# zwpku/colvars-finder

Measured on AMD Instinct MI355X. Metric: MD frames/sec through EigenFunctionTask train step, higher is better.
Workload: dtype f32; 1 GPU; BASELINE config 3: alanine-dipeptide-shaped EigenFunctionTask, generator mode, k=3, 22 atoms, align+position features d_r=66, nets [66,20,20,20,1], diag_coeff, Adam; frames_per_gpu=100000, batch_per_gpu=20000, global_batch=20000, parallelism=dp1 (frames sharded; all-reduce of batch sums + flat gradient)

## Files before the change

### colvars-finder_amd/csrc/ef16_back.hip

```cpp
#include "ef16_common.hpp"

namespace {

struct Back16Args {
  int k;
  int64_t B;
  int64_t n_tiles;
  int64_t T;
  const float* w_lag;
};
struct Back16Nets {
  int D;
  int n_params;
  int base[CVF_MAX_NETS];
};
template <int H, int NH>
__host__ __device__ constexpr int net_w_off(int l, int hd) { return l == 0 ? 0 : hd + H + (l - 1) * (H * H + H); }
template <int H, int NH>
__host__ __device__ constexpr int net_b_off(int l, int hd) { return net_w_off<H, NH>(l, hd) + (l == 0 ? hd : l == NH ? H : H * H); }

template <int H, int NH, bool MULTI, bool GEN>
__global__ __launch_bounds__(256, 4) void ef16_back_kernel(Back16Args args, Back16Nets nets, const float* __restrict__ theta,
                                                            const float* __restrict__ packed, const float* __restrict__ w,
                                                            const float* __restrict__ feat, const float* __restrict__ y_tiled,
                                                            const float* __restrict__ q_tiled, const double* __restrict__ coef,
                                                            float* __restrict__ slab, int32_t* __restrict__ step,
                                                            const float* __restrict__ saved) {
  constexpr int RT = Hid<H>::RT, NG = Hid<H>::NG;
  constexpr int RTO = (H + 15) / 16;
  constexpr int CTH = (H + 1 + 15) / 16;
  constexpr int NT = 256, WPB = 4;
  constexpr bool TAIL4 = RTO == 2 && H % 16 >= 1 && H % 16 <= 4;
  constexpr int kRows = 2 * H + 2 * (H + 1) + 16;
  __shared__ __attribute__((aligned(16))) float IMG[kRows * kPitch];
  __shared__ float PART[4 * (H + 1)];
  extern __shared__ float GI[];
  float* SA1 = IMG;
  float* SA2 = SA1 + H * kPitch;
  float* SB1 = SA2 + H * kPitch;
  float* SB2 = SB1 + (H + 1) * kPitch;
  const int tid = threadIdx.x;
  const int wave = __builtin_amdgcn_readfirstlane(tid >> 6);
  int lane = tid & 63, col, q, row16, r0, fo, rowf;
  auto derive_lane = [&]() {
    col = lane & 15, q = lane >> 4, row16 = col, r0 = 4 * q;
    fo = 16 * wave + col;
    rowf = 4 * col + q;
  };
  derive_lane();
  static_assert(H % 4 == 0, "a lane's four rows of a gradient tile are inside the layer together (emit_tile)");
  const int net = blockIdx.y;
  int k = args.k;
  int D = nets.D, HD, c0, nfeat, ncol, CTM;
  bool strip;
  PackLayout L;
  auto derive = [&]() {
    const int CT1 = (D + 1 + 15) / 16;
    HD = H * D;
    c0 = 16 * (CT1 - 1), nfeat = D - c0, ncol = nfeat + 1;
    strip = ncol <= 4;
    CTM = strip ? CT1 - 1 : CT1;
    L = pack_layout(H, NH, D);
  };
  derive();
  const int gbase = nets.base[net];
  const int gspan = net_b_off<H, NH>(NH, HD) + 1;
  float* out = slab + (int64_t)blockIdx.x * nets.n_params + gbase;

  {
    static_assert((kRows * kPitch) % 4 == 0, "IMG is zeroed in 16-byte pieces");
    float4* img4 = reinterpret_cast<float4*>(IMG);
    for (int i = tid; i < kRows * kPitch / 4; i += NT) img4[i] = float4{0.0f, 0.0f, 0.0f, 0.0f};
  }
  if (MULTI)
    for (int i = tid; i < gspan; i += NT) GI[i] = 0.0f;
  lds_barrier();
  if (tid < 64) SB1[H * kPitch + tid] = 1.0f;

  const URows pk = urows(packed + (int64_t)net * L.per_net, L.per_net, lane);
  float wl[RT][4];
  load_hid_const_u<H>(urows(theta + gbase + net_w_off<H, NH>(NH, HD), H, q), wl);
  const float one[1] = {1.0f};

  const __amdgpu_buffer_rsrc_t out_rs = __builtin_amdgcn_make_buffer_rsrc(out, 0, gspan * 4, 0x00020000);
  constexpr int kDead = 0x7fff0000;
  auto emit_tile = [&](int l, int n_in, int rt, int ct, const f32x4& acc) {
    const int wo = net_w_off<H, NH>(l, HD), bo = net_b_off<H, NH>(l, HD);
    const int i = 16 * ct + row16;
    int ob = 16 * rt + r0;
    asm volatile("" : "+v"(ob));
    const bool isb = i == n_in, live = ob < H && i <= n_in;
    const int idx0 = isb ? bo + ob : wo + ob * n_in + i, stride = isb ? 1 : n_in;
    const int off0 = live ? idx0 * 4 : kDead;
#pragma unroll
    for (int r = 0; r < 4; ++r) {
      const float av = acc[r];
      if (MULTI) {
        if (live) GI[idx0 + r * stride] += av;
      } else {
        __builtin_amdgcn_raw_buffer_store_b32(__builtin_bit_cast(int, av), out_rs, off0 + r * stride * 4, 0, 0);
      }
    }
  };
  auto outer2 = [&](const float* A1, const float* B1, const float* A2, const float* B2, int rt, int ct) {
    f32x4 acc = {0.0f, 0.0f, 0.0f, 0.0f};
    acc = outer_half(A1, B1, rt, ct, lane, acc);
    if constexpr (GEN) acc = outer_half(A2, B2, rt, ct, lane, acc);
    return acc;
  };

  auto emit_entry = [&](bool live, int idx, float v) {
    if (MULTI) {
      if (live) GI[idx] += v;
    } else {
      __builtin_amdgcn_raw_buffer_store_b32(__builtin_bit_cast(int, v), out_rs, live ? idx * 4 : kDead, 0, 0);
    }
  };
  auto emit_last = [&]() {
    if (wave == WPB - 1) {
      int i = lane;
      asm volatile("" : "+v"(i));
      const bool live = i <= H;
      const float v = strip_total(PART + (live ? i : H), H + 1);
      emit_entry(live, i < H ? net_w_off<H, NH>(NH, HD) + i : net_b_off<H, NH>(NH, HD), v);
    }
  };
  auto emit_strip = [&]() {
    if (strip && 64 * wave < 4 * H) {
      int e = tid;
      asm volatile("" : "+v"(e));
      const int o = e >> 2, c = e & 3;
      const bool live = o < H && c < ncol;
      const float v = strip_total(SB1 + (o < H ? e : 0), 4 * H);
      emit_entry(live, c < nfeat ? o * D + c0 + c : HD + o, v);
    }
  };

  int64_t tile = blockIdx.x;
  do {
    if constexpr (MULTI) {
      asm volatile("" : "+s"(D), "+s"(k));
      derive();
      asm volatile("" : "+v"(lane));
      derive_lane();
    }
    CVF_STAMP(8);
    double crow[CVF_MAX_NETS];
#pragma unroll
    for (int j = 0; j < CVF_MAX_NETS; ++j) crow[j] = coef[k + net * k + (j < k ? j : k - 1)];
    double gS1n = coef[net], gEtn = coef[k + k * k + net];
    double gS1ln = GEN ? 0.0 : coef[2 * k + k * k + net], gS2ln = GEN ? 0.0 : coef[3 * k + k * k + net];
    __builtin_amdgcn_sched_barrier(0);
    const bool lagged = !GEN && tile >= args.T;
    const int64_t t0 = lagged ? tile - args.T : tile;
    const int64_t frame = t0 * CVF_TILE + fo;
    const bool valid = frame < args.B;
    const float wraw = w[valid ? frame : args.B - 1];
    float yb[CVF_MAX_NETS];
#pragma unroll
    for (int j = 0; j < CVF_MAX_NETS; ++j) yb[j] = y_tiled[(t0 * k + (j < k ? j : k - 1)) * CVF_TILE + fo];
    float ylag = 0.0f, wlraw = 0.0f;
    if constexpr (!GEN) {
      ylag = y_tiled[((args.T + t0) * k + net) * CVF_TILE + fo];
      wlraw = args.w_lag[valid ? frame : args.B - 1];
    }
    const URows sv = urows(saved + (tile * k + net) * (int64_t)(kHand<NH>() * NG * 256) + wave * 64, kHand<NH>() * NG * 256 - wave * 64, lane);
    Vec<H, 1> h[NH], e[NH > 1 ? NH - 1 : 1], t[NH];
#pragma unroll
    for (int l = 0; l < NH; ++l) {
#pragma unroll
      for (int rt = 0; rt < RT; ++rt) h[l].v[rt][0] = f32x4{0.0f, 0.0f, 0.0f, 0.0f};
#pragma unroll
      for (int g = 0; g < NG; ++g) h[l].v[g >> 2][0][g & 3] = sv.ld((l * NG + g) * 256);
    }
    if constexpr (GEN) {
#pragma unroll
      for (int l = 0; l + 1 < NH; ++l) {
#pragma unroll
        for (int rt = 0; rt < RT; ++rt) e[l].v[rt][0] = f32x4{0.0f, 0.0f, 0.0f, 0.0f};
#pragma unroll
        for (int g = 0; g < NG; ++g) e[l].v[g >> 2][0][g & 3] = sv.ld(((NH + l) * NG + g) * 256);
      }
#pragma unroll
      for (int rt = 0; rt < RT; ++rt) t[0].v[rt][0] = f32x4{0.0f, 0.0f, 0.0f, 0.0f};
#pragma unroll
      for (int g = 0; g < NG; ++g) t[0].v[g >> 2][0][g & 3] = sv.ld(((2 * NH - 1) * NG + g) * 256);
    }
    HFrag<H> ffr[NH > 1 ? NH - 1 : 1];
    if constexpr (GEN) {
#pragma unroll
      for (int l = 1; l < NH; ++l) load_hfrag_u<H>(ffr[l - 1], pk, L.fh(l));
    }
    const float* f_tile = feat + tile * (int64_t)D * CVF_TILE;
    const float* q_tile = GEN ? q_tiled + (tile * k + net) * (int64_t)D * CVF_TILE : nullptr;
    const float wb = valid ? wraw : 0.0f;
    float alpha, gamma = 0.0f;
    float ynet = 0.0f;
#pragma unroll
    for (int j = 0; j < CVF_MAX_NETS; ++j)
      if (j == net) ynet = yb[j];
#pragma unroll
    for (int j = 0; j < CVF_MAX_NETS; ++j) asm volatile("" : "+s"(crow[j]));
    asm volatile("" : "+s"(gS1n), "+s"(gEtn));
    if constexpr (!GEN) asm volatile("" : "+s"(gS1ln), "+s"(gS2ln));
    if (GEN || !lagged) {
      double a = gS1n;
#pragma unroll
      for (int j = 0; j < CVF_MAX_NETS; ++j)
        if (j < k) a += (j == net ? 2.0 : 1.0) * crow[j] * (double)yb[j];
      alpha = (float)((double)wb * a);
      if constexpr (GEN) gamma = (float)(2.0 * (double)wb * gEtn);
      else alpha = (float)((double)wb * a - 2.0 * (double)wb * gEtn * ((double)ylag - (double)ynet));
    } else {
      const double wlg = valid ? (double)wlraw : 0.0;
      alpha = (float)(wlg * (gS1ln + 2.0 * gS2ln * (double)ylag) + 2.0 * (double)wb * gEtn * ((double)ylag - (double)ynet));
    }
    CVF_STAMP(9);
    if constexpr (GEN) {
#pragma unroll
      for (int rt = 0; rt < RT; ++rt)
#pragma unroll
        for (int r = 0; r < 4; ++r) t[0].v[rt][0][r] *= gamma;
#pragma unroll
      for (int l = 1; l < NH; ++l) {
        Vec<H, 1> td;
        tangent_of<H, 1>(td, h[l - 1], t[l - 1]);
        init_bias<H, 1>(t[l], nullptr, q);
        hidden_mul<H, 1>(t[l], ffr[l - 1], td);
      }
    }
    CVF_STAMP(11);
    {
      const float pick = strip_rows<H>([&](int rt, int r) {
        const float hv = h[NH - 1].v[rt][0][r];
        if constexpr (GEN) return fmaf(alpha, hv, (1.0f - hv * hv) * t[NH - 1].v[rt][0][r]);
        else return alpha * hv;
      }, col);
      const float sa = row_sumf16(alpha);
      if (col < NG && rowf < H) PART[wave * (H + 1) + rowf] = pick;
      if (lane == 0) PART[wave * (H + 1) + H] = sa;
    }
    CVF_STAMP(12);
    Vec<H, 1> hbar;
#pragma unroll
    for (int rt = 0; rt < RT; ++rt)
#pragma unroll
      for (int r = 0; r < 4; ++r) hbar.v[rt][0][r] = alpha * wl[rt][r];
    HFrag<H> tfl;
    float4 bA[4], bB[4];
    float xs[3] = {0.0f, 0.0f, 0.0f}, qs[3] = {0.0f, 0.0f, 0.0f};
    auto request = [&](float4 (&dst)[4], const float* src_tile, int ct) {
      const int i = 16 * ct + row16;
      const float4* p = reinterpret_cast<const float4*>(src_tile + (int64_t)(i < D ? i : D - 1) * CVF_TILE + 4 * q);
#pragma unroll
      for (int j = 0; j < 4; ++j) dst[j] = p[4 * j];
    };
    auto request_step = [&](int l) {
      if (l > 0) {
        load_hfrag_u<H>(tfl, pk, L.th(l));
      } else {
        if (strip) {
#pragma unroll
          for (int c = 0; c < 3; ++c)
            if (c < nfeat) {
              xs[c] = f_tile[(int64_t)(c0 + c) * CVF_TILE + fo];
              if constexpr (GEN) qs[c] = q_tile[(int64_t)(c0 + c) * CVF_TILE + fo];
            }
        }
        request(bA, f_tile, wave);
        if constexpr (GEN) request(bB, q_tile, wave);
      }
    };
    request_step(NH - 1);
#pragma unroll
    for (int l = NH - 1; l >= 0; --l) {
      CVF_STAMP(13 + (NH - 1 - l));
      Vec<H, 1> zbar, dl;
#pragma unroll
      for (int rt = 0; rt < RT; ++rt)
#pragma unroll
        for (int r = 0; r < 4; ++r) {
          const float hv = h[l].v[rt][0][r];
          const float om = 1.0f - hv * hv;
          if constexpr (GEN) {
            const float ev = (l == NH - 1) ? wl[rt][r] : e[l < NH - 1 ? l : 0].v[rt][0][r];
            const float hb = fmaf(-2.0f * hv * t[l].v[rt][0][r], ev, hbar.v[rt][0][r]);
            dl.v[rt][0][r] = ev * om;
            zbar.v[rt][0][r] = om * hb;
          } else {
            zbar.v[rt][0][r] = om * hbar.v[rt][0][r];
          }
        }
      store_image<H, 1, false>(SA1, zbar, one, lane, fo);
      if constexpr (GEN) {
        const float sc[1] = {l == 0 ? gamma : 1.0f};
        store_image<H, 1, true>(SA2, dl, sc, lane, fo);
      }
      if (l > 0) {
        store_image<H, 1, false>(SB1, h[l - 1], one, lane, fo);
        if constexpr (GEN) {
          Vec<H, 1> td;
          tangent_of<H, 1>(td, h[l - 1], t[l - 1]);
          store_image<H, 1, false>(SB2, td, one, lane, fo);
        }
        __syncthreads();
        init_bias<H, 1>(hbar, nullptr, q);
        hidden_mul<H, 1>(hbar, tfl, zbar);
        request_step(l - 1);
        if constexpr (TAIL4) {
          const int role = (wave + 2 * (l & 1)) & 3;
          if (role == 0) {
            emit_tile(l, H, 0, 0, outer2(SA1, SB1, SA2, SB2, 0, 0));
          } else {
            const int g = col >> 2, m = lane & 3;
            const int wo = net_w_off<H, NH>(l, HD), bo = net_b_off<H, NH>(l, HD);
            auto job = [&](int arow, int brow, int o, int i, bool live) {
              f32x4 acc = {0.0f, 0.0f, 0.0f, 0.0f};
              acc = outer_half44(SA1, arow, SB1, brow, lane, acc);
              if constexpr (GEN) acc = outer_half44(SA2, arow, SB2, brow, lane, acc);
              const float v = rows_sum_scatter(acc);
              asm volatile("" : "+v"(o));
              live = live && o < H && i <= H;
              emit_entry(live, i < H ? wo + o * H + i : bo + o, v);
            };
            const bool low = role == 1;
            const int cb = role == 3 ? 20 : 16;
            job(low ? 16 + m : 4 * g + m, low ? 4 * g + m : cb + m, low ? 16 + q : 4 * g + q, low ? 4 * g + m : cb + m, true);
            if (low) job(16 + m, 16 + 4 * (g & 1) + m, 16 + q, 16 + 4 * (g & 1) + m, g < 2);
          }
        } else {
          for (int pr = wave; pr < RTO * CTH; pr += WPB) {
            const int rt = pr / CTH, ct = pr - rt * CTH;
            emit_tile(l, H, rt, ct, outer2(SA1, SB1, SA2, SB2, rt, ct));
          }
        }
        if (l == NH - 1) emit_last();
        __syncthreads();
      } else {
        if (strip) {
#pragma unroll
          for (int c = 0; c < 4; ++c) {
            if (c < ncol) {
              const float xv = c == nfeat ? 1.0f : xs[c < 3 ? c : 2];
              const float qv = c == nfeat ? 0.0f : gamma * qs[c < 3 ? c : 2];
              const float pick = strip_rows<H>([&](int rt, int r) {
                if constexpr (GEN) return fmaf(zbar.v[rt][0][r], xv, dl.v[rt][0][r] * qv);
                else return zbar.v[rt][0][r] * xv;
              }, col);
              if (col < NG && rowf < H) SB1[(wave * H + rowf) * 4 + c] = pick;
            }
          }
        }
        __syncthreads();
        auto half0 = [&](f32x4 (&acc)[RTO], const float* SA, const float4 (&b)[4], int ct, int rt0, int rstep, bool ones) {
          const int i = 16 * ct + row16;
          const float pad = (ones && i == D) ? 1.0f : 0.0f;
#pragma unroll
          for (int rt = 0; rt < RTO; ++rt) {
            if (rt >= rt0 && (rt - rt0) % rstep == 0) {
              const float4* a1 = reinterpret_cast<const float4*>(SA + (16 * rt + row16) * kPitch + 4 * q);
              float4 av[4];
#pragma unroll
              for (int j = 0; j < 4; ++j) av[j] = a1[4 * j];
#pragma unroll
              for (int j = 0; j < 4; ++j) {
                acc[rt] = mfma4(av[j].x, i < D ? b[j].x : pad, acc[rt]);
                acc[rt] = mfma4(av[j].y, i < D ? b[j].y : pad, acc[rt]);
                acc[rt] = mfma4(av[j].z, i < D ? b[j].z : pad, acc[rt]);
                acc[rt] = mfma4(av[j].w, i < D ? b[j].w : pad, acc[rt]);
              }
            }
          }
        };
        const int extra = (CTM - WPB) * RTO;
        f32x4 acc[RTO];
#pragma unroll
        for (int rt = 0; rt < RTO; ++rt) acc[rt] = f32x4{0.0f, 0.0f, 0.0f, 0.0f};
        auto tail0 = [&](f32x4& tacc, const float* SA, const float4 (&b)[4], int ct, bool ones) {
          const int i = 16 * ct + row16;
          const float pad = (ones && i == D) ? 1.0f : 0.0f;
          const float4* a1 = reinterpret_cast<const float4*>(SA + (16 + (lane & 3)) * kPitch + 4 * q);
          float4 av[4];
#pragma unroll
          for (int j = 0; j < 4; ++j) av[j] = a1[4 * j];
#pragma unroll
          for (int j = 0; j < 4; ++j) {
            tacc = mfma1(av[j].x, i < D ? b[j].x : pad, tacc);
            tacc = mfma1(av[j].y, i < D ? b[j].y : pad, tacc);
            tacc = mfma1(av[j].z, i < D ? b[j].z : pad, tacc);
            tacc = mfma1(av[j].w, i < D ? b[j].w : pad, tacc);
          }
        };
        if (wave < CTM) {
          f32x4 tacc = {0.0f, 0.0f, 0.0f, 0.0f};
          half0(acc, SA1, bA, wave, 0, TAIL4 ? RTO : 1, true);
          if constexpr (TAIL4) tail0(tacc, SA1, bA, wave, true);
          if (wave < extra) request(bA, f_tile, WPB + wave / RTO);
          if constexpr (GEN) {
            half0(acc, SA2, bB, wave, 0, TAIL4 ? RTO : 1, false);
            if constexpr (TAIL4) tail0(tacc, SA2, bB, wave, false);
          }
#pragma unroll
          for (int rt = 0; rt < (TAIL4 ? 1 : RTO); ++rt) emit_tile(0, D, rt, wave, acc[rt]);
          if constexpr (TAIL4) {
            const float v = rows_sum_scatter(tacc);
            int o = 16 + q;
            asm volatile("" : "+v"(o));
            const int i = 16 * wave + row16;
            const bool isw = o < H && i < D, isb = o < H && i == D;
            emit_entry(isw || isb, isw ? o * D + i : HD + (o < H ? o : 0), v);
          }
        }
        for (int pr = wave; pr < extra; pr += WPB) {
          const int ct = WPB + pr / RTO, rt = pr % RTO;
          if (pr != wave || wave >= CTM) request(bA, f_tile, ct);
          if constexpr (GEN) request(bB, q_tile, ct);
#pragma unroll
          for (int r_ = 0; r_ < RTO; ++r_) acc[r_] = f32x4{0.0f, 0.0f, 0.0f, 0.0f};
          half0(acc, SA1, bA, ct, rt, RTO, true);
          if constexpr (GEN) half0(acc, SA2, bB, ct, rt, RTO, false);
#pragma unroll
          for (int r_ = 0; r_ < RTO; ++r_)
            if (r_ == rt) emit_tile(0, D, r_, ct, acc[r_]);
        }
        emit_strip();
        if (NH == 1) emit_last();
        __syncthreads();
      }
    }
    tile += gridDim.x;
  } while (MULTI && tile < args.n_tiles);
  CVF_STAMP(17);
  if (MULTI) {
    __syncthreads();
    for (int i = tid; i < gspan; i += NT) out[i] = GI[i];
  }
  if (step != nullptr && blockIdx.x == 0 && blockIdx.y == 0 && tid == 0) *step += 1;
  CVF_STAMP(18);
}

}

extern "C" int64_t cvf_ef16_backward_slab_rows(int64_t n_tiles) { return n_tiles < 1024 ? n_tiles : 1024; }

static int ef16_backward_impl(const cvf_ef_cfg* cfg, const cvf_mlp_desc* mlp, const float* theta, const float* packed,
                              int64_t B, const float* w, const float* w_lag, const float* feat_tiled, const float* y_tiled,
                              const float* q_tiled, const double* coef, float* slab, int32_t* step_count, const float* saved,
                              void* stream) {
  const bool transfer = cfg != nullptr && cfg->lag_idx > 0;
  CVF_REQUIRE(cfg && mlp && theta && packed && w && feat_tiled && y_tiled && (transfer ? w_lag != nullptr : q_tiled != nullptr) && coef &&
              slab && saved && B > 0, "cvf_ef16_backward: bad argument");
  CVF_REQUIRE(cfg->k == mlp->n_nets, "cvf_ef16_backward: cfg.k must equal the number of nets");
  int H, NH;
  CVF_REQUIRE(ef16_shape(mlp, &H, &NH), "cvf_ef16_backward: unsupported net shape");
  CVF_REQUIRE(mlp->dims[0] <= 8 * 16 - 1, "cvf_ef16_backward: first layer wider than the column-tile schedule covers");
  const int span = mlp->b_off[0][NH] + 1 - mlp->w_off[0][0];
  int covered = 0;
  for (int n = 0; n < mlp->n_nets; ++n) {
    CVF_REQUIRE(mlp->b_off[n][NH] + 1 - mlp->w_off[n][0] == span, "cvf_ef16_backward: nets are not laid out contiguously");
    for (int l = 0; l <= NH; ++l)
      CVF_REQUIRE(mlp->w_off[n][l] >= mlp->w_off[n][0] && mlp->b_off[n][l] < mlp->w_off[n][0] + span,
                  "cvf_ef16_backward: nets are not laid out contiguously");
    covered += span;
  }
  CVF_REQUIRE(covered == mlp->n_params, "cvf_ef16_backward: flat buffer holds parameters outside the nets");
  for (int n = 0; n < mlp->n_nets; ++n)
    for (int l = 0; l <= NH; ++l) {
      CVF_REQUIRE(mlp->b_off[n][l] == mlp->w_off[n][l] + mlp->dims[l] * mlp->dims[l + 1],
                  "cvf_ef16_backward: net %d, layer %d: the bias does not follow the weight", n, l);
      CVF_REQUIRE(l == NH || mlp->w_off[n][l + 1] == mlp->b_off[n][l] + mlp->dims[l + 1],
                  "cvf_ef16_backward: net %d: layer %d does not follow layer %d", n, l + 1, l);
    }
  Back16Nets nets;
  nets.D = mlp->dims[0];
  nets.n_params = mlp->n_params;
  for (int n = 0; n < CVF_MAX_NETS; ++n) nets.base[n] = n < mlp->n_nets ? mlp->w_off[n][0] : 0;
  Back16Args a;
  a.k = cfg->k;
  a.B = B;
  a.T = cvf_ntiles(B);
  a.n_tiles = transfer ? 2 * a.T : a.T;
  a.w_lag = w_lag;
  const int64_t G = cvf_ef16_backward_slab_rows(a.n_tiles);
  const bool launched = ef16_dispatch(H, NH, [&](auto h_, auto nh_) {
    constexpr int kH = decltype(h_)::value, kNH = decltype(nh_)::value;
    auto go = [&](auto kernel, size_t lds) {
      hipLaunchKernelGGL(kernel, dim3((unsigned)G, cfg->k), dim3(256), lds, (hipStream_t)stream, a, nets, theta, packed, w, feat_tiled,
                         y_tiled, q_tiled, coef, slab, step_count, saved);
    };
    const size_t gi = (size_t)span * sizeof(float);
    if (transfer) {
      if (a.n_tiles > G) go(ef16_back_kernel<kH, kNH, true, false>, gi);
      else go(ef16_back_kernel<kH, kNH, false, false>, 0);
    } else {
      if (a.n_tiles > G) go(ef16_back_kernel<kH, kNH, true, true>, gi);
      else go(ef16_back_kernel<kH, kNH, false, true>, 0);
    }
  });
  CVF_REQUIRE(launched, "cvf_ef16_backward: no kernel instance for hidden width %d x %d layers", H, NH);
  return cvf_check_launch("ef16_back_kernel");
}

extern "C" int cvf_ef16_backward(const cvf_ef_cfg* cfg, const cvf_mlp_desc* mlp, const float* theta, const float* packed,
                                 int64_t B, const float* w, const float* feat_tiled, const float* y_tiled, const float* q_tiled,
                                 const double* coef, float* slab, int32_t* step_count, const float* saved, void* stream) {
  CVF_REQUIRE(cfg && cfg->lag_idx == 0, "cvf_ef16_backward: generator mode (transfer-operator mode: cvf_ef16_backward_transfer)");
  return ef16_backward_impl(cfg, mlp, theta, packed, B, w, nullptr, feat_tiled, y_tiled, q_tiled, coef, slab, step_count, saved, stream);
}


extern "C" int cvf_ef16_backward_transfer(const cvf_ef_cfg* cfg, const cvf_mlp_desc* mlp, const float* theta, const float* packed,
                                          int64_t B, const float* w, const float* w_lag, const float* feat_tiled,
                                          const float* y_tiled, const double* coef, float* slab, int32_t* step_count,
                                          const float* saved, void* stream) {
  CVF_REQUIRE(cfg && cfg->lag_idx > 0, "cvf_ef16_backward_transfer: transfer-operator mode (cfg.lag_idx > 0)");
  return ef16_backward_impl(cfg, mlp, theta, packed, B, w, w_lag, feat_tiled, y_tiled, nullptr, coef, slab, step_count, saved, stream);
}
```

### colvars-finder_amd/csrc/ef16_common.hpp

```cpp
#pragma once
#include "cvf_metric.hpp"
#include "ef_frag.hpp"
#include <stdlib.h>
#include <type_traits>


namespace {

constexpr int kU = 16;
constexpr int kImgP = 76;
constexpr int kAuxP = 21;
constexpr int kMaxRows16 = 16384;
template <int NH>
__host__ __device__ constexpr int kHand() { return 2 * NH; }

__device__ __forceinline__ float quad_sumf16(float v) {
  v += dpp_movf<0xB1, 0xf>(v);
  v += dpp_movf<0x4E, 0xf>(v);
  return v;
}
__device__ __forceinline__ double quad_sumd16(double v) {
  v += dpp_movd<0xB1, 0xf>(v);
  v += dpp_movd<0x4E, 0xf>(v);
  return v;
}

__device__ __forceinline__ float row_sumf16(float v) {
  v = quad_sumf16(v);
  v += dpp_movf<0x141, 0xf>(v);
  v += dpp_movf<0x140, 0xf>(v);
  return v;
}
template <int H, class F>
__device__ __forceinline__ float strip_rows(F&& val, int col) {
  float pick = 0.0f;
#pragma unroll
  for (int j = 0; j < Hid<H>::NG; ++j) {
    const float s = row_sumf16(val(j >> 2, j & 3));
    pick = col == j ? s : pick;
  }
  return pick;
}
__device__ __forceinline__ float strip_total(const float* P, int stride) {
  return ((P[0] + P[stride]) + P[2 * stride]) + P[3 * stride];
}

__device__ __forceinline__ float rows_sum_scatter(const f32x4& x) {
  auto swap_add = [](auto swapped) {
    const unsigned a = swapped[0], b = swapped[1];
    return __builtin_bit_cast(float, a) + __builtin_bit_cast(float, b);
  };
  const float x0 = x[0], x1 = x[1], x2 = x[2], x3 = x[3];
  const float s02 = swap_add(__builtin_amdgcn_permlane32_swap(__builtin_bit_cast(unsigned, x0), __builtin_bit_cast(unsigned, x2), false, false));
  const float s13 = swap_add(__builtin_amdgcn_permlane32_swap(__builtin_bit_cast(unsigned, x1), __builtin_bit_cast(unsigned, x3), false, false));
  return swap_add(__builtin_amdgcn_permlane16_swap(__builtin_bit_cast(unsigned, s02), __builtin_bit_cast(unsigned, s13), false, false));
}

struct Front16Lds {
  int ref, a, aux, w, rs, y, e, feat, g, total;
};
__host__ __device__ inline Front16Lds front16_lds(int nc, int nal, int k) {
  Front16Lds L;
  const int stride = x_tile_stride(nc);
  L.ref = kU * stride;
  L.a = L.ref + 3 * nal;
  L.aux = (L.a + nc + 3) & ~3;
  L.w = L.aux + ((kU * kAuxP + 3) & ~3);
  L.rs = L.w + kU;
  L.y = L.rs + 4;
  L.e = L.y + k * kU;
  L.feat = L.e + k * kU;
  L.g = L.feat + kU * kImgP;
  L.total = L.g + k * kU * kImgP;
  return L;
}

bool ef16_shape(const cvf_mlp_desc* m, int* H, int* NH) {
  if (m->n_layers < 2 || m->n_layers > 4 || m->dims[m->n_layers] != 1) return false;
  *H = m->dims[1];
  *NH = m->n_layers - 1;
  for (int l = 1; l < m->n_layers; ++l)
    if (m->dims[l] != *H) return false;
  for (int l = 0; l < m->n_layers; ++l)
    if (m->act[l] != (l + 1 < m->n_layers ? 1 : 0)) return false;
  return true;
}

template <class F>
bool ef16_dispatch(int H, int NH, F&& f) {
#define EF_CASE(H_, NH_)                                                        \
  if (H == H_ && NH == NH_) {                                                   \
    f(std::integral_constant<int, H_>{}, std::integral_constant<int, NH_>{});   \
    return true;                                                                \
  }
#ifdef CVF_DEV_SHAPES
  EF_CASE(20, 3)
#else
  EF_CASE(8, 1) EF_CASE(8, 2) EF_CASE(8, 3)
  EF_CASE(12, 1) EF_CASE(12, 2) EF_CASE(12, 3)
  EF_CASE(16, 1) EF_CASE(16, 2) EF_CASE(16, 3)
  EF_CASE(20, 1) EF_CASE(20, 2) EF_CASE(20, 3)
  EF_CASE(24, 2) EF_CASE(24, 3)
  EF_CASE(32, 2) EF_CASE(32, 3)
#endif
#undef EF_CASE
  return false;
}

}
```

### colvars-finder_amd/csrc/ef16_front.hip

```cpp
#include "ef16_front_kernel.hpp"


extern "C" int cvf_ef16_supported(const cvf_mlp_desc* mlp, const cvf_pp_desc* pp) {
  int H, NH;
  if (!mlp || !pp || !ef16_shape(mlp, &H, &NH) || getenv("CVF_NO_EF16")) return 0;
  if (!ef16_dispatch(H, NH, [](auto, auto) {})) return 0;
  const int fast = CVF_PP_ALIGN_CONTIG | CVF_PP_PURE_POSITION;
  if (pp->mode != CVF_PP_ALIGN || pp->align_w || (pp->flags & fast) != fast || pp->n_align > pp->n_rec || pp->n_align < 3) return 0;
  if (pp->d_r != 3 * pp->n_rec || pp->d_r != mlp->dims[0] || pp->d_r > 72 || pp->n_coord > 192 || pp->n_coord < pp->d_r) return 0;
  if (mlp->n_nets < 1 || mlp->n_nets > CVF_MAX_NETS) return 0;
  return (size_t)front16_lds(pp->n_coord, pp->n_align, mlp->n_nets).total * sizeof(float) <= 64 * 1024;
}

extern "C" int64_t cvf_ef16_scratch_doubles(int64_t B, int k) {
  const int64_t units = 4 * cvf_ntiles(B);
  const int64_t rows = units <= kMaxRows16 ? units : 0;
  return rows * cvf_ef_nstats(k, 1) + cvf_ef_stats_scratch_doubles(k, 1);
}

extern "C" int64_t cvf_ef16_rows(int64_t B) {
  const int64_t units = 4 * cvf_ntiles(B);
  return units <= kMaxRows16 ? units : 0;
}
extern "C" int cvf_ef16_finish(const cvf_ef_cfg* cfg, int64_t B, const double* scratch, double* stats, double* loss_vec, double* coef,
                               void* stream) {
  CVF_REQUIRE(cfg && scratch && stats && cvf_ef16_rows(B) > 0, "cvf_ef16_finish: bad argument");
  CVF_REQUIRE(loss_vec == nullptr || coef != nullptr, "cvf_ef16_finish: loss_vec without coef");
  return cvf_ef_stats_finish_impl(cfg, (int)cvf_ef16_rows(B), 1, scratch, stats, loss_vec, coef, (hipStream_t)stream);
}

extern "C" int cvf_ef16_finish_dp(const cvf_ef_cfg* cfg, int64_t B, const double* scratch, double* stats, double* loss_vec, double* coef,
                                  void* p2p_comm, void* stream) {
  CVF_REQUIRE(cfg && scratch && stats && loss_vec && coef && cvf_ef16_rows(B) > 0, "cvf_ef16_finish_dp: bad argument");
  const P2PLL* ll = cvf_p2p_ll(p2p_comm, 0);
  if (ll == nullptr) return -1;
  return cvf_ef_stats_finish_ll(cfg, (int)cvf_ef16_rows(B), 1, scratch, stats, loss_vec, coef, (hipStream_t)stream, ll);
}

extern "C" int64_t cvf_ef16_saved_floats(const cvf_mlp_desc* mlp, int64_t n_tiles) {
  int H, NH;
  if (!mlp || !ef16_shape(mlp, &H, &NH)) return 0;
  return n_tiles * mlp->n_nets * (2 * NH) * (int64_t)((H + 3) / 4) * 256;
}

extern "C" int cvf_ef16_front(const cvf_mlp_desc* mlp, const float* theta, const float* packed, float* feat_tiled,
                              const cvf_pp_desc* pp, const float* x, int64_t B, const float* a, float* y_tiled, float* saved,
                              float* q_tiled, float* e_tiled, const cvf_ef_cfg* cfg, const float* w, double* scratch, double* stats,
                              double* loss_vec, double* coef, void* stream) {
  return ef16_front_go<false>("cvf_ef16_front", mlp, theta, packed, feat_tiled, pp, x, B, a, y_tiled, saved, q_tiled, e_tiled, cfg, w, scratch,
                              stats, loss_vec, coef, nullptr, stream);
}

extern "C" int cvf_ef16_front_iso(const cvf_mlp_desc* mlp, const float* theta, const float* packed, float* feat_tiled,
                                  const cvf_pp_desc* pp, const float* x, int64_t B, const float* a, float* y_tiled, float* saved,
                                  float* q_tiled, float* e_tiled, const cvf_ef_cfg* cfg, const float* w, double* scratch, double* stats,
                                  double* loss_vec, double* coef, void* stream) {
  return ef16_front_go<false>("cvf_ef16_front_iso", mlp, theta, packed, feat_tiled, pp, x, B, a, y_tiled, saved, q_tiled, e_tiled, cfg, w,
                              scratch, stats, loss_vec, coef, nullptr, stream, true);
}


static int ef16_front_transfer_impl(const cvf_mlp_desc* mlp, const float* theta, const float* packed, float* feat_tiled,
                                    const cvf_pp_desc* pp, const float* x, const float* x_lag, int64_t B, float* y_tiled, float* saved,
                                    const float* w, const float* w_lag, double* rows_out, void* stream, const char* what) {
  CVF_REQUIRE(pp && pp->mode != CVF_PP_FACTORED, "%s: takes coordinates, not CVF_PP_FACTORED records", what);
  CVF_REQUIRE(cvf_ef16_supported(mlp, pp), "%s: shape not covered (cvf_ef16_supported() == 0)", what);
  CVF_REQUIRE(theta && packed && feat_tiled && x && x_lag && y_tiled && saved && B > 0, "%s: bad argument", what);
  int H, NH;
  ef16_shape(mlp, &H, &NH);
  const int k = mlp->n_nets;
  const int64_t T = cvf_ntiles(B), units = 4 * T;
  CVF_REQUIRE(2 * units < (int64_t)1 << 31, "%s: batch too large for one launch", what);
  const bool paired = rows_out != nullptr || getenv("CVF_EF16_UNPAIRED") == nullptr;
  const size_t lds1 = ((size_t)front16_lds(pp->n_coord, pp->n_align, k).g + 16) * sizeof(float);
  const int upb = paired ? ef16_units_per_wg(units, k, lds1) : 1;
  const size_t lds = lds1 * upb;
  ef16_dispatch(H, NH, [&](auto h_, auto nh_) {
    constexpr int kH = decltype(h_)::value, kNH = decltype(nh_)::value;
    auto kernel = ef16_front_kernel<kH, kNH, 0, true>;
    if (lds > 48 * 1024) (void)hipFuncSetAttribute((const void*)kernel, hipFuncAttributeMaxDynamicSharedMemorySize, (int)lds);
    hipLaunchKernelGGL(kernel, dim3((unsigned)(paired ? (units + upb - 1) / upb : 2 * units)), dim3(64 * k * upb), lds, (hipStream_t)stream, *mlp,
                       theta, packed, *pp, x, B, (const float*)nullptr, w, feat_tiled, y_tiled, saved, (float*)nullptr, (float*)nullptr,
                       rows_out, upb | (paired ? 256 : 0), x_lag, units, w_lag, (const float*)nullptr);
  });
  return cvf_check_launch("ef16_front_kernel");
}

extern "C" int cvf_ef16_front_transfer(const cvf_mlp_desc* mlp, const float* theta, const float* packed, float* feat_tiled,
                                       const cvf_pp_desc* pp, const float* x, const float* x_lag, int64_t B, float* y_tiled,
                                       float* saved, void* stream) {
  return ef16_front_transfer_impl(mlp, theta, packed, feat_tiled, pp, x, x_lag, B, y_tiled, saved, nullptr, nullptr, nullptr, stream,
                                  "cvf_ef16_front_transfer");
}

extern "C" int64_t cvf_ef16_transfer_rows(int64_t B, int k) { return k >= 1 ? cvf_ef16_rows(B) : 0; }
extern "C" int cvf_ef16_front_transfer_rows(const cvf_mlp_desc* mlp, const float* theta, const float* packed, float* feat_tiled,
                                            const cvf_pp_desc* pp, const float* x, const float* x_lag, int64_t B, float* y_tiled,
                                            float* saved, const float* w, const float* w_lag, double* scratch, void* stream) {
  CVF_REQUIRE(w && w_lag && scratch && mlp && cvf_ef16_transfer_rows(B, mlp->n_nets) > 0, "cvf_ef16_front_transfer_rows: bad argument");
  return ef16_front_transfer_impl(mlp, theta, packed, feat_tiled, pp, x, x_lag, B, y_tiled, saved, w, w_lag, scratch, stream,
                                  "cvf_ef16_front_transfer_rows");
}
```

### colvars-finder_amd/csrc/ef16_front_kernel.hpp

```cpp
#pragma once
#include "ef16_common.hpp"
#include "cvf_p2p.hpp"

namespace {
constexpr int kRowsUnit = kU * kAuxP;
static_assert(kRowsUnit % 4 == 0, "a unit's alignment rows are staged as 16-byte pieces");

template <bool kTransfer>
__device__ __forceinline__ void ef16_align_unit(const float* my, const float* refL, const int nal, const int lane, float* auxL,
                                                float* rsL) {
  const int f = lane >> 2, p = lane & 3;
  double acc[15];
#pragma unroll
  for (int i = 0; i < 15; ++i) acc[i] = 0.0;
#pragma unroll 2
  for (int b = p; b < nal; b += 4) {
    const double x0 = (double)my[3 * b], x1 = (double)my[3 * b + 1], x2 = (double)my[3 * b + 2];
    const double r0 = (double)refL[3 * b], r1 = (double)refL[3 * b + 1], r2 = (double)refL[3 * b + 2];
    acc[0] += x0; acc[1] += x1; acc[2] += x2;
    acc[3] = fma(x0, r0, acc[3]); acc[4] = fma(x0, r1, acc[4]); acc[5] = fma(x0, r2, acc[5]);
    acc[6] = fma(x1, r0, acc[6]); acc[7] = fma(x1, r1, acc[7]); acc[8] = fma(x1, r2, acc[8]);
    acc[9] = fma(x2, r0, acc[9]); acc[10] = fma(x2, r1, acc[10]); acc[11] = fma(x2, r2, acc[11]);
    acc[12] += r0; acc[13] += r1; acc[14] += r2;
  }
#pragma unroll
  for (int i = 0; i < 15; ++i) acc[i] = quad_sumd16(acc[i]);
  const double inv = fast_rcp((double)nal);
  const double cd[3] = {acc[0] * inv, acc[1] * inv, acc[2] * inv};
  double Hm[3][3];
#pragma unroll
  for (int i = 0; i < 3; ++i)
#pragma unroll
    for (int j = 0; j < 3; ++j) Hm[i][j] = fma(-cd[i], acc[12 + j], acc[3 + 3 * i + j]);
  KabschOut ko;
  if constexpr (kTransfer) {
    kabsch_from_H<false>(Hm, ko);
#pragma unroll
    for (int i = 0; i < 6; ++i) ko.Kinv[i] = 0.0f;
  } else {
    kabsch_from_H<true>(Hm, ko);
  }
  const Centre c = centre_of(cd);
  const float av[kAuxP] = {ko.R[0], ko.R[1], ko.R[2], ko.R[3], ko.R[4], ko.R[5], ko.R[6], ko.R[7], ko.R[8], c.hi[0], c.hi[1], c.hi[2],
                           ko.Kinv[0], ko.Kinv[1], ko.Kinv[2], ko.Kinv[3], ko.Kinv[4], ko.Kinv[5], c.lo[0], c.lo[1], c.lo[2]};
#pragma unroll
  for (int i = 0; i < kAuxP; ++i)
    if ((i & 3) == p) auxL[f * kAuxP + i] = av[i];
  if (lane < 3) rsL[lane] = (float)(lane == 0 ? acc[12] : lane == 1 ? acc[13] : acc[14]);
}

__device__ __forceinline__ V3 ef16_feature(const float* my, const int at, const Centre& c, const float* R) {
  return row_times(centred(my, at, c), R);
}

template <int H, int NH, int NIT, bool ALLAL, bool ROWS = false>
__global__ __launch_bounds__(1024, 4) void ef16_front_kernel(cvf_mlp_desc mlp, const float* __restrict__ theta,
                                                             const float* __restrict__ packed, cvf_pp_desc pp,
                                                             const float* __restrict__ x, int64_t B,
                                                             const float* __restrict__ a, const float* __restrict__ w,
                                                             float* __restrict__ feat_tiled, float* __restrict__ y_tiled,
                                                             float* __restrict__ saved, float* __restrict__ q_tiled,
                                                             float* __restrict__ e_tiled, double* __restrict__ partial, int launch,
                                                             const float* __restrict__ x_lag, int64_t units_x,
                                                             const float* __restrict__ w_lag, const float* __restrict__ rows) {
  static_assert(!ROWS || NIT > 0, "alignment rows: generator instances only");
  constexpr int RT = Hid<H>::RT, NG = Hid<H>::NG, SMAX = 18, CTMAX = 5;
  constexpr bool kTransfer = NIT == 0;
  extern __shared__ __attribute__((aligned(16))) float lds_all[];
  const int upb = launch & 0xff;
  const int k = mlp.n_nets, D = mlp.dims[0];
  const int wave_b = __builtin_amdgcn_readfirstlane((int)threadIdx.x >> 6);
  const int usub = upb > 1 ? wave_b / k : 0;
  const int wave = wave_b - usub * k;
  const int tid = (int)threadIdx.x - usub * (64 * k), lane_in = tid & 63;
  const int nthreads = upb > 1 ? 64 * k : (int)blockDim.x, nw = nthreads >> 6;
  const int net = wave;
  const int64_t ublock = (int64_t)blockIdx.x * upb + usub;
  const bool paired = kTransfer && x_lag != nullptr && ((launch >> 8) & 1) != 0;
  const bool iso = !kTransfer && ((launch >> 9) & 1) != 0;
  const int nc = pp.n_coord, nal = pp.n_align, N = pp.n_rec;
  const int stride = x_tile_stride(nc);
  const Front16Lds Lo = front16_lds(nc, nal, k);
  float* lds = lds_all + usub * (kTransfer ? Lo.g + 16 : Lo.total);
  const int64_t n_ublock = (kTransfer && !paired) ? 2 * units_x : units_x;
  const int64_t ub = ublock < n_ublock ? ublock : n_ublock - 1;
  const float* const x_first = x;
  const float* const w_first = w;
  auto run_pass = [&](const int pass) __attribute__((always_inline)) {
  const int lane = lane_in;
  const PackLayout L = pack_layout(H, NH, D);
  const URows pk = urows(packed + (int64_t)net * L.per_net, L.per_net, lane);
  const int S = (D + 3) >> 2, CT = (D + 15) >> 4;
  float a0[SMAX][RT];
  float bias[NH][RT][4];
  const int q_ = lane >> 4;
  auto request_a0 = [&]() {
#pragma unroll
    for (int s = 0; s < SMAX; ++s) {
      const int se = s < S ? s : S - 1;
#pragma unroll
      for (int rt = 0; rt < RT; ++rt) a0[s][rt] = pk.ld(L.f0() + (se * RT + rt) * 64);
    }
  };
  auto request_bias0 = [&]() { load_hid_const_u<H>(urows(theta + mlp.b_off[net][0], H, q_), bias[0]); };
  auto request_layer0 = [&]() {
    request_a0();
    request_bias0();
  };
  const bool lagged = x_lag != nullptr && (paired ? pass == 1 : ub >= units_x);
  const int64_t unit = (lagged && !paired) ? ub - units_x : ub;
  const int64_t tile = (unit >> 2) + (lagged ? (units_x >> 2) : 0);
  const int sub = (int)(unit & 3);
  x = lagged ? x_lag : x_first;
  w = lagged ? w_lag : w_first;
  float* xt = lds;
  float* refL = lds + Lo.ref;
  float* aL = lds + Lo.a;
  float* auxL = lds + Lo.aux;
  float* wL = (kTransfer && pass == 1) ? lds + Lo.g : lds + Lo.w;
  float* rsL = lds + Lo.rs;
  float* yL = lds + Lo.y + (kTransfer ? pass * (k * kU) : 0);
  float* eL = lds + Lo.e;
  float* featI = lds + Lo.feat;
  float* gI = lds + Lo.g + net * (kU * kImgP);
  const int f = lane >> 2, p = lane & 3;
  const int col = lane & 15, q = lane >> 4;

  CVF_STAMP(20);
  float bf0[SMAX];
  if constexpr (ROWS) {
    constexpr int n4r = kRowsUnit / 4;
    const float4* rsrc = reinterpret_cast<const float4*>(rows + unit * (int64_t)kRowsUnit);
    const float4 row_a = rsrc[tid < n4r ? tid : n4r - 1];
    const float4 row_b = rsrc[tid + nthreads < n4r ? tid + nthreads : n4r - 1];
    const float rs_in = rows[units_x * (int64_t)kRowsUnit + (tid < 3 ? tid : 2)];
    const bool plain = stride == nc && (unit + 1) * kU <= B && (reinterpret_cast<uintptr_t>(x) & 15) == 0;
    const int n4 = (kU * nc) >> 2;
    const float4* xsrc = reinterpret_cast<const float4*>(x + unit * (int64_t)(kU * nc));
    const float4* xs = plain ? xsrc : rsrc;
    const int nx = plain ? n4 : 1;
    float4 cx0 = {0.0f, 0.0f, 0.0f, 0.0f}, cx1 = cx0;
    if (!iso) {
      cx0 = xs[tid < nx ? tid : nx - 1];
      cx1 = xs[tid + nthreads < nx ? tid + nthreads : nx - 1];
    }
    const int nt = 3 * nal + nc, jt = tid < nt ? tid : nt - 1;
    const bool in_a = jt >= 3 * nal && a != nullptr;
    const float tv_ld = *(in_a ? a + (jt - 3 * nal) : pp.ref_c + (jt < 3 * nal ? jt : 0));
    const float tv = (jt < 3 * nal || in_a) ? tv_ld : 0.0f;
    const int64_t frame = unit * kU + (tid < kU ? tid : kU - 1);
    const float wv_ld = *(w != nullptr ? w + (frame < B ? frame : B - 1) : rows);
    const float wv = (w != nullptr && frame < B) ? wv_ld : 0.0f;
    {
      const float* ft = feat_tiled + tile * (int64_t)D * CVF_TILE + kU * sub + col;
#pragma unroll
      for (int s = 0; s < SMAX; ++s) {
        const int kf = 4 * (s < S ? s : S - 1) + q;
        bf0[s] = ft[(kf < D ? kf : D - 1) * CVF_TILE];
      }
    }
    request_a0();
    float4* adst = reinterpret_cast<float4*>(auxL);
    if (tid < n4r) adst[tid] = row_a;
    if (tid + nthreads < n4r) adst[tid + nthreads] = row_b;
    if (tid < 3) rsL[tid] = rs_in;
    if (iso) {
    } else if (plain) {
      float4* dst = reinterpret_cast<float4*>(xt);
      if (tid < n4) dst[tid] = cx0;
      if (tid + nthreads < n4) dst[tid + nthreads] = cx1;
      for (int v = tid + 2 * nthreads; v < n4; v += nthreads) dst[v] = xsrc[v];
    } else {
      load_x_tile<6>(x, B, nc, unit, xt, tid, nthreads, kU);
    }
    if (tid < nt) refL[tid] = tv;
    for (int j = tid + nthreads; j < nt; j += nthreads) refL[j] = j < 3 * nal ? pp.ref_c[j] : (a != nullptr ? a[j - 3 * nal] : 0.0f);
    if (tid < kU) wL[tid] = wv;
    request_bias0();
  } else {
  if (stride == nc && (unit + 1) * kU <= B && (reinterpret_cast<uintptr_t>(x) & 15) == 0) {
    const float4* src = reinterpret_cast<const float4*>(x + unit * (int64_t)(kU * nc));
    float4* dst = reinterpret_cast<float4*>(xt);
    const int n4 = (kU * nc) >> 2;
    for (int v = tid; v < n4; v += nthreads) dst[v] = src[v];
  } else {
    load_x_tile<6>(x, B, nc, unit, xt, tid, nthreads, kU);
  }
  for (int j = tid; j < 3 * nal + nc; j += nthreads) refL[j] = j < 3 * nal ? pp.ref_c[j] : (a != nullptr ? a[j - 3 * nal] : 0.0f);
  if (tid < kU) {
    const int64_t frame = unit * kU + tid;
    wL[tid] = (w != nullptr && frame < B) ? w[frame] : 0.0f;
  }
  if (wave != 0) request_layer0();
  __syncthreads();
  }
  const float* my = xt + f * stride;
  CVF_STAMP(21);

  if constexpr (!ROWS) {
    if (wave == 0) {
      ef16_align_unit<kTransfer>(my, refL, nal, lane, auxL, rsL);
      request_layer0();
    }
    lds_barrier();
  }
  CVF_STAMP(22);

  if constexpr (!ROWS) {
    float R[9];
    const float* ar = auxL + f * kAuxP;
#pragma unroll
    for (int i = 0; i < 9; ++i) R[i] = ar[i];
    Centre c;
#pragma unroll
    for (int i = 0; i < 3; ++i) {
      c.hi[i] = ar[9 + i];
      c.lo[i] = ar[18 + i];
    }
    for (int at = p + 4 * wave; at < N; at += 4 * nw) {
      const V3 al = ef16_feature(my, at, c, R);
      float* fi = featI + f * kImgP + 3 * at;
      fi[0] = al.x;
      fi[1] = al.y;
      fi[2] = al.z;
    }
    lds_barrier();
  }
  CVF_STAMP(23);

  Vec<H, 1> h[NH];
  auto set_bias = [&](Vec<H, 1>& X, const float (&b)[RT][4]) {
#pragma unroll
    for (int rt = 0; rt < RT; ++rt)
#pragma unroll
      for (int r = 0; r < 4; ++r) X.v[rt][0][r] = b[rt][r];
  };
  set_bias(h[0], bias[0]);
  {
    float bf[SMAX];
    float* fr = featI + col * kImgP;
    static_assert(4 * (SMAX - 1) + 3 < kImgP, "the ROWS twins' feature copy stays inside a frame's row of the image");
    unsigned own = 0u;
    if constexpr (ROWS) {
      if (iso) {
        const int P = nw >= 8 ? 8 : nw >= 4 ? 4 : nw >= 2 ? 2 : 1;
        own = (P == 8 ? 0x10101u : P == 4 ? 0x11111u : P == 2 ? 0x15555u : 0x3ffffu) << (wave & (P - 1));
      }
    }
#pragma unroll
    for (int s = 0; s < SMAX; ++s) {
      const int kf = 4 * (s < S ? s : S - 1) + q;
      if constexpr (ROWS) bf[s] = bf0[s];
      else bf[s] = fr[kf < D ? kf : D - 1];
    }
    HFrag<H> hf[NH > 1 ? NH - 1 : 1];
#pragma unroll
    for (int l = 1; l < NH; ++l) {
      load_hfrag_u<H>(hf[l - 1], pk, L.fh(l));
      load_hid_const_u<H>(urows(theta + mlp.b_off[net][l], H, q), bias[l]);
    }
#pragma unroll
    for (int s = 0; s < SMAX; ++s) {
      if (s < S) {
#pragma unroll
        for (int rt = 0; rt < RT; ++rt) h[0].v[rt][0] = mfma4(a0[s][rt], bf[s], h[0].v[rt][0]);
        if constexpr (ROWS) {
          if ((own >> s) & 1u) fr[q + 4 * s] = bf[s];
        }
      }
    }
    CVF_STAMP(24);
    tanh_inplace<H, 1>(h[0]);
#pragma unroll
    for (int l = 1; l < NH; ++l) {
      set_bias(h[l], bias[l]);
      hidden_mul<H, 1>(h[l], hf[l - 1], h[l - 1]);
      tanh_inplace<H, 1>(h[l]);
    }
  }
  float wl[RT][4];
  load_hid_const_u<H>(urows(theta + mlp.w_off[net][NH], H, q), wl);
  const float bL = theta[mlp.b_off[net][NH]];
  HFrag<H> tf[NH > 1 ? NH - 1 : 1];
#pragma unroll
  for (int l = 1; l < NH; ++l) load_hfrag_u<H>(tf[l - 1], pk, L.th(l));

  const URows sv = urows(saved + (tile * k + net) * (int64_t)(kHand<NH>() * NG * 256) + sub * 64, kHand<NH>() * NG * 256 - sub * 64, lane);
  {
    float part = 0.0f;
#pragma unroll
    for (int rt = 0; rt < RT; ++rt)
#pragma unroll
      for (int r = 0; r < 4; ++r) part = fmaf(wl[rt][r], h[NH - 1].v[rt][0][r], part);
    const float yv = sum_over_q(part) + bL;
    yL[net * kU + col] = yv;
    y_tiled[(tile * k + net) * CVF_TILE + kU * sub + col] = yv;
  }
  CVF_STAMP(25);
  if constexpr (kTransfer) {
#pragma unroll
    for (int l = 0; l < NH; ++l)
#pragma unroll
      for (int g = 0; g < NG; ++g) sv.st((l * NG + g) * 256, h[l].v[g >> 2][0][g & 3]);
    float* ft = feat_tiled + tile * (int64_t)D * CVF_TILE + kU * sub + f;
    const float* fi = featI + f * kImgP;
#pragma unroll 1
    for (int j = p + 4 * wave; j < D; j += 4 * nw) ft[j * CVF_TILE] = fi[j];
    return;
  } else {

  {
    float t0[CTMAX][NG];
#pragma unroll
    for (int rt = 0; rt < CTMAX; ++rt)
#pragma unroll
      for (int s = 0; s < NG; ++s) t0[rt][s] = pk.ld(L.t0() + ((rt < CT ? rt : CT - 1) * NG + s) * 64);
    Vec<H, 1> d;
#pragma unroll
    for (int rt = 0; rt < RT; ++rt)
#pragma unroll
      for (int r = 0; r < 4; ++r) {
        const float hv = h[NH - 1].v[rt][0][r];
        d.v[rt][0][r] = wl[rt][r] * (1.0f - hv * hv);
      }
    Vec<H, 1> ev[NH > 1 ? NH - 1 : 1];
#pragma unroll
    for (int l = NH - 1; l >= 1; --l) {
      init_bias<H, 1>(ev[l - 1], nullptr, q);
      hidden_mul<H, 1>(ev[l - 1], tf[l - 1], d);
      tangent_of<H, 1>(d, h[l - 1], ev[l - 1]);
    }
#pragma unroll
    for (int rt = 0; rt < CTMAX; ++rt) {
      if (rt < CT) {
        f32x4 acc = {0.0f, 0.0f, 0.0f, 0.0f};
#pragma unroll
        for (int s = 0; s < NG; ++s) acc = mfma4(t0[rt][s], d.v[s >> 2][0][s & 3], acc);
        if (16 * rt + 4 * q < D) *reinterpret_cast<float4*>(gI + col * kImgP + 16 * rt + 4 * q) = float4{acc[0], acc[1], acc[2], acc[3]};
      }
    }
#pragma unroll
    for (int l = 0; l < NH; ++l)
#pragma unroll
      for (int g = 0; g < NG; ++g) sv.st((l * NG + g) * 256, h[l].v[g >> 2][0][g & 3]);
#pragma unroll
    for (int l = 1; l < NH; ++l)
#pragma unroll
      for (int g = 0; g < NG; ++g) sv.st(((NH + l - 1) * NG + g) * 256, ev[l - 1].v[g >> 2][0][g & 3]);
  }
  if constexpr (ROWS) lds_barrier();
  CVF_STAMP(26);
  asm volatile("s_waitcnt lgkmcnt(0)" ::: "memory");

  float f0b[SMAX][RT];
  {
    const float* ar = auxL + f * kAuxP;
    float* Ul = gI + f * kImgP;
    V3 gv[NIT];
    if (iso) {
    const float* Fl = featI + f * kImgP;
    V3 gsum = v3(0.0f, 0.0f, 0.0f), tau = v3(0.0f, 0.0f, 0.0f);
#pragma unroll
    for (int it = 0; it < NIT; ++it) {
      int at = p + 4 * it;
      asm volatile("" : "+v"(at));
      const bool last = it == NIT - 1;
      const int ac = (last && at >= N) ? N - 1 : at;
      const float lv = (last && at >= N) ? 0.0f : 1.0f;
      gv[it] = v3(Ul[3 * ac], Ul[3 * ac + 1], Ul[3 * ac + 2]);
      const V3 fb = v3(Fl[3 * ac], Fl[3 * ac + 1], Fl[3 * ac + 2]);
      const V3 gm = last ? lv * gv[it] : gv[it];
      gsum = gsum + gm;
      tau.x = fmaf(gm.y, fb.z, fmaf(-gm.z, fb.y, tau.x));
      tau.y = fmaf(gm.z, fb.x, fmaf(-gm.x, fb.z, tau.y));
      tau.z = fmaf(gm.x, fb.y, fmaf(-gm.y, fb.x, tau.z));
    }
    CVF_STAMP(27);
    gsum = v3(quad_sumf16(gsum.x), quad_sumf16(gsum.y), quad_sumf16(gsum.z));
    tau = v3(quad_sumf16(tau.x), quad_sumf16(tau.y), quad_sumf16(tau.z));
    float Kinv[6];
#pragma unroll
    for (int i = 0; i < 6; ++i) Kinv[i] = ar[12 + i];
    const V3 s = sym_times(Kinv, tau);
    const float inv_nal = 1.0f / (float)nal;
    const V3 gbar = inv_nal * gsum;
    float E = 0.0f;
    V3 usum = v3(0.0f, 0.0f, 0.0f), tau2 = v3(0.0f, 0.0f, 0.0f);
#pragma unroll
    for (int it = 0; it < NIT; ++it) {
      int at = p + 4 * it;
      asm volatile("" : "+v"(at));
      const bool last = it == NIT - 1;
      const int ac = (last && at >= N) ? N - 1 : at;
      const float lv = (last && at >= N) ? 0.0f : 1.0f;
      const float ma = ALLAL ? 1.0f : (ac < nal ? 1.0f : 0.0f);
      const int ar_ = ALLAL ? ac : (ac < nal ? ac : 0);
      V3 rf = v3(refL[3 * ar_], refL[3 * ar_ + 1], refL[3 * ar_ + 2]);
      if (!ALLAL) rf = ma * rf;
      const V3 sh = ALLAL ? gbar : ma * gbar;
      V3 G;
      G.x = fmaf(s.y, rf.z, fmaf(-s.z, rf.y, gv[it].x - sh.x));
      G.y = fmaf(s.z, rf.x, fmaf(-s.x, rf.z, gv[it].y - sh.y));
      G.z = fmaf(s.x, rf.y, fmaf(-s.y, rf.x, gv[it].z - sh.z));
      const V3 u = aL[3 * ac] * G;
      gv[it] = u;
      const bool masked = last || !ALLAL;
      const V3 ue = last ? lv * u : u;
      E = fmaf(ue.x, G.x, fmaf(ue.y, G.y, fmaf(ue.z, G.z, E)));
      const V3 um = masked ? (ma * lv) * u : u;
      usum = usum + um;
      tau2.x = fmaf(rf.y, um.z, fmaf(-rf.z, um.y, tau2.x));
      tau2.y = fmaf(rf.z, um.x, fmaf(-rf.x, um.z, tau2.y));
      tau2.z = fmaf(rf.x, um.y, fmaf(-rf.y, um.x, tau2.z));
    }
    CVF_STAMP(28);
    E = quad_sumf16(E);
    usum = v3(quad_sumf16(usum.x), quad_sumf16(usum.y), quad_sumf16(usum.z));
    tau2 = v3(quad_sumf16(tau2.x), quad_sumf16(tau2.y), quad_sumf16(tau2.z));
    const V3 rsum = v3(rsL[0], rsL[1], rsL[2]);
    eL[net * kU + f] = E;
    e_tiled[(tile * k + net) * CVF_TILE + kU * sub + f] = E;
    const V3 ubar = inv_nal * usum;
    tau2.x = fmaf(-rsum.y, ubar.z, fmaf(rsum.z, ubar.y, tau2.x));
    tau2.y = fmaf(-rsum.z, ubar.x, fmaf(rsum.x, ubar.z, tau2.y));
    tau2.z = fmaf(-rsum.x, ubar.y, fmaf(rsum.y, ubar.x, tau2.z));
    const V3 om = sym_times(Kinv, tau2);
    CVF_STAMP(31);
#pragma unroll
    for (int it = 0; it < NIT; ++it) {
      int at = p + 4 * it;
      asm volatile("" : "+v"(at));
      const int ac = (it == NIT - 1 && at >= N) ? N - 1 : at;
      const V3 fb = v3(Fl[3 * ac], Fl[3 * ac + 1], Fl[3 * ac + 2]);
      V3 qv;
      qv.x = fmaf(fb.y, om.z, fmaf(-fb.z, om.y, gv[it].x - ubar.x));
      qv.y = fmaf(fb.z, om.x, fmaf(-fb.x, om.z, gv[it].y - ubar.y));
      qv.z = fmaf(fb.x, om.y, fmaf(-fb.y, om.x, gv[it].z - ubar.z));
      gv[it] = qv;
      Ul[3 * ac] = qv.x;
      Ul[3 * ac + 1] = qv.y;
      Ul[3 * ac + 2] = qv.z;
    }
    } else {
    float R[9];
#pragma unroll
    for (int i = 0; i < 9; ++i) R[i] = ar[i];
    const Centre c = centre_of(ar[9], ar[10], ar[11]);
    V3 gsum = v3(0.0f, 0.0f, 0.0f);
    Outer3 Mo = {{{0.0f, 0.0f}, {0.0f, 0.0f}, {0.0f, 0.0f}}, {0.0f, 0.0f, 0.0f}};
#pragma unroll
    for (int it = 0; it < NIT; ++it) {
      int at = p + 4 * it;
      asm volatile("" : "+v"(at));
      const bool last = it == NIT - 1;
      const int ac = (last && at >= N) ? N - 1 : at;
      const float lv = (last && at >= N) ? 0.0f : 1.0f;
      gv[it] = v3(Ul[3 * ac], Ul[3 * ac + 1], Ul[3 * ac + 2]);
      const V3 gm = last ? lv * gv[it] : gv[it];
      gsum = gsum + gm;
      outer_acc(Mo, centred(my, ac, c), gm);
    }
    CVF_STAMP(27);
    gsum = v3(quad_sumf16(gsum.x), quad_sumf16(gsum.y), quad_sumf16(gsum.z));
    const V3 sump = mat_times(R, gsum);
    float M[9];
    outer_to_array(Mo, M);
#pragma unroll
    for (int i = 0; i < 9; ++i) M[i] = quad_sumf16(M[i]);
    float T[9], Z[9];
#pragma unroll
    for (int i = 0; i < 3; ++i)
#pragma unroll
      for (int j = 0; j < 3; ++j) T[3 * i + j] = R[i] * M[j] + R[3 + i] * M[3 + j] + R[6 + i] * M[6 + j];
    float Kinv[6];
#pragma unroll
    for (int i = 0; i < 6; ++i) Kinv[i] = ar[12 + i];
    const V3 s = sym_times(Kinv, v3(T[7] - T[5], T[2] - T[6], T[3] - T[1]));
#pragma unroll
    for (int i = 0; i < 3; ++i) {
      Z[3 * i + 0] = R[3 * i + 1] * s.z - R[3 * i + 2] * s.y;
      Z[3 * i + 1] = -R[3 * i + 0] * s.z + R[3 * i + 2] * s.x;
      Z[3 * i + 2] = R[3 * i + 0] * s.y - R[3 * i + 1] * s.x;
    }
    const float inv_nal = 1.0f / (float)nal;
    const V3 shift = inv_nal * sump;
    const MatCols Rc = mat_cols(R), Zc = mat_cols(Z);
    f2 E2 = {0.0f, 0.0f};
    float Ez = 0.0f;
    f2 usum_xy = {0.0f, 0.0f};
    float usum_z = 0.0f;
    Outer3 dHo = {{{0.0f, 0.0f}, {0.0f, 0.0f}, {0.0f, 0.0f}}, {0.0f, 0.0f, 0.0f}};
#pragma unroll
    for (int it = 0; it < NIT; ++it) {
      int at = p + 4 * it;
      asm volatile("" : "+v"(at));
      const bool last = it == NIT - 1;
      const int ac = (last && at >= N) ? N - 1 : at;
      const float lv = (last && at >= N) ? 0.0f : 1.0f;
      const float ma = ALLAL ? 1.0f : (ac < nal ? 1.0f : 0.0f);
      const int ar_ = ALLAL ? ac : (ac < nal ? ac : 0);
      V3 rf = v3(refL[3 * ar_], refL[3 * ar_ + 1], refL[3 * ar_ + 2]);
      if (!ALLAL) rf = ma * rf;
      f2 Gxy = ALLAL ? f2{-shift.x, -shift.y} : f2{-ma * shift.x, -ma * shift.y};
      float Gz = ALLAL ? -shift.z : -ma * shift.z;
      mat_times_acc(Rc, gv[it], Gxy, Gz);
      mat_times_acc(Zc, rf, Gxy, Gz);
      const f2 uxy = f2{aL[3 * ac], aL[3 * ac + 1]} * Gxy;
      const float uz = aL[3 * ac + 2] * Gz;
      gv[it] = v3(uxy.x, uxy.y, uz);
      const bool masked = last || !ALLAL;
      const float m = ma * lv;
      const f2 uxm = masked ? m * uxy : uxy;
      const float uzm = masked ? m * uz : uz;
      E2 = fma2(last ? lv * uxy : uxy, Gxy, E2);
      Ez = fmaf(last ? lv * uz : uz, Gz, Ez);
      usum_xy += uxm; usum_z += uzm;
      outer_acc(dHo, v3(uxm.x, uxm.y, uzm), rf);
    }
    CVF_STAMP(28);
    const float E = quad_sumf16((E2.x + E2.y) + Ez);
    const V3 usum = v3(quad_sumf16(usum_xy.x), quad_sumf16(usum_xy.y), quad_sumf16(usum_z));
    const V3 rsum = v3(rsL[0], rsL[1], rsL[2]);
    float dH[9];
    outer_to_array(dHo, dH);
#pragma unroll
    for (int i = 0; i < 9; ++i) dH[i] = quad_sumf16(dH[i]);
    eL[net * kU + f] = E;
    e_tiled[(tile * k + net) * CVF_TILE + kU * sub + f] = E;
    const V3 ubar = inv_nal * usum;
    dH[0] -= ubar.x * rsum.x; dH[1] -= ubar.x * rsum.y; dH[2] -= ubar.x * rsum.z;
    dH[3] -= ubar.y * rsum.x; dH[4] -= ubar.y * rsum.y; dH[5] -= ubar.y * rsum.z;
    dH[6] -= ubar.z * rsum.x; dH[7] -= ubar.z * rsum.y; dH[8] -= ubar.z * rsum.z;
#pragma unroll
    for (int i = 0; i < 3; ++i)
#pragma unroll
      for (int j = 0; j < 3; ++j) T[3 * i + j] = R[i] * dH[j] + R[3 + i] * dH[3 + j] + R[6 + i] * dH[6 + j];
    asm volatile("" ::: "memory");
#pragma unroll
    for (int i = 0; i < 6; ++i) Kinv[i] = ar[12 + i];
    const V3 om = sym_times(Kinv, v3(T[7] - T[5], T[2] - T[6], T[3] - T[1]));
    float dR[9];
#pragma unroll
    for (int i = 0; i < 3; ++i) {
      dR[3 * i + 0] = R[3 * i + 1] * om.z - R[3 * i + 2] * om.y;
      dR[3 * i + 1] = -R[3 * i + 0] * om.z + R[3 * i + 2] * om.x;
      dR[3 * i + 2] = R[3 * i + 0] * om.y - R[3 * i + 1] * om.x;
    }
    CVF_STAMP(31);
    const MatRows Rr = mat_rows(R), dRr = mat_rows(dR);
#pragma unroll
    for (int it = 0; it < NIT; ++it) {
      int at = p + 4 * it;
      asm volatile("" : "+v"(at));
      const int ac = (it == NIT - 1 && at >= N) ? N - 1 : at;
      f2 qxy = {0.0f, 0.0f};
      float qz = 0.0f;
      row_times_acc(Rr, gv[it] - ubar, qxy, qz);
      row_times_acc(dRr, centred(my, ac, c), qxy, qz);
      gv[it] = v3(qxy.x, qxy.y, qz);
      Ul[3 * ac] = qxy.x;
      Ul[3 * ac + 1] = qxy.y;
      Ul[3 * ac + 2] = qz;
    }
    }
    CVF_STAMP(32);
    asm volatile("" ::: "memory");
#pragma unroll
    for (int s_ = 0; s_ < SMAX; ++s_) {
      const int se = s_ < S ? s_ : S - 1;
#pragma unroll
      for (int rt = 0; rt < RT; ++rt) f0b[s_][rt] = pk.ld(L.f0() + (se * RT + rt) * 64);
    }
    {
      asm volatile("s_waitcnt lgkmcnt(0)" ::: "memory");
      Vec<H, 1> sv0;
      init_bias<H, 1>(sv0, nullptr, q);
      const float* qr = gI + col * kImgP;
#pragma unroll
      for (int s = 0; s < SMAX; ++s) {
        if (s < S) {
          const int kf = 4 * s + q;
          const float b = qr[kf < D ? kf : D - 1];
#pragma unroll
          for (int rt = 0; rt < RT; ++rt) sv0.v[rt][0] = mfma4(f0b[s][rt], b, sv0.v[rt][0]);
        }
      }
#pragma unroll
      for (int g = 0; g < NG; ++g) sv.st(((2 * NH - 1) * NG + g) * 256, sv0.v[g >> 2][0][g & 3]);
    }
    CVF_STAMP(33);
    float* qt = q_tiled + (tile * k + net) * (int64_t)D * CVF_TILE + kU * sub + f;
#pragma unroll
    for (int it = 0; it < NIT; ++it) {
      int at = p + 4 * it;
      asm volatile("" : "+v"(at));
      const int ac = (it == NIT - 1 && at >= N) ? N - 1 : at;
      qt[(3 * ac) * CVF_TILE] = gv[it].x;
      qt[(3 * ac + 1) * CVF_TILE] = gv[it].y;
      qt[(3 * ac + 2) * CVF_TILE] = gv[it].z;
    }
  }
  CVF_STAMP(34);
  if constexpr (!ROWS) {
    float* ft = feat_tiled + tile * (int64_t)D * CVF_TILE + kU * sub + f;
    const float* fi = featI + f * kImgP;
#pragma unroll 1
    for (int j = p + 4 * wave; j < D; j += 4 * nw) ft[j * CVF_TILE] = fi[j];
  }
  CVF_STAMP(29);
  if (partial == nullptr) return;
  lds_barrier();

  if (wave == 0) {
    typedef double f64x4 __attribute__((ext_vector_type(4)));
    const int np = CVF_NPAIR(k);
    const int i = lane & 15, kq = lane >> 4;
    f64x4 d1 = {0.0, 0.0, 0.0, 0.0}, d2 = {0.0, 0.0, 0.0, 0.0};
    const float* yrow = yL + (i >= 1 && i <= k ? i - 1 : 0) * kU;
    const float* erow = eL + (i < k ? i : 0) * kU;
#pragma unroll
    for (int s_ = 0; s_ < 4; ++s_) {
      const int fr = 4 * s_ + kq;
      const double wb = (double)wL[fr];
      const double yv = (double)yrow[fr];
      const double a1 = i == 0 ? 1.0 : (i <= k ? yv : 0.0);
      const double b = i == 0 ? wb : (i <= k ? wb * yv : 0.0);
      const double a2 = i < k ? (double)erow[fr] : 0.0;
      d1 = __builtin_amdgcn_mfma_f64_16x16x4f64(a1, b, d1, 0, 0, 0);
      d2 = __builtin_amdgcn_mfma_f64_16x16x4f64(a2, b, d2, 0, 0, 0);
    }
    const int cj = lane & 15;
    const int64_t G = units_x;
#pragma unroll
    for (int r = 0; r < 4; ++r) {
      const int ri = (lane >> 4) + 4 * r;
      int t = -1;
      if (ri == 0 && cj <= k) t = cj;
      else if (ri >= 1 && ri <= cj && cj <= k) {
        const int a_ = ri - 1, b_ = cj - 1;
        t = 1 + k + a_ * k - (a_ * (a_ - 1)) / 2 + (b_ - a_);
      }
      if (t >= 0) partial[t * G + unit] = d1[r];
      if (cj == 0 && ri < k) partial[(1 + k + np + ri) * G + unit] = d2[r];
    }
  }
  CVF_STAMP(30);
  }
  };
  run_pass(0);
  if constexpr (kTransfer) {
    if (!paired) return;
    run_pass(1);
    if (partial == nullptr) return;
    const int lane = lane_in;
    const int64_t unit = ub;
    lds_barrier();
    if (wave == 0) {
      typedef double f64x4 __attribute__((ext_vector_type(4)));
      const int np = CVF_NPAIR(k);
      const int i = lane & 15, kq = lane >> 4;
      const float* y0 = lds + Lo.y;
      const float* y1 = y0 + k * kU;
      const float* w0 = lds + Lo.w;
      const float* w1 = lds + Lo.g;
      f64x4 d1 = {0.0, 0.0, 0.0, 0.0}, d2 = {0.0, 0.0, 0.0, 0.0}, d3 = {0.0, 0.0, 0.0, 0.0};
      const int yi = (i >= 1 && i <= k ? i - 1 : 0) * kU, ti = (i < k ? i : 0) * kU;
#pragma unroll
      for (int s_ = 0; s_ < 4; ++s_) {
        const int fr = 4 * s_ + kq;
        const double wb = (double)w0[fr], wl_ = (double)w1[fr];
        const double yv = (double)y0[yi + fr], ylv = (double)y1[yi + fr];
        const double a1 = i == 0 ? 1.0 : (i <= k ? yv : 0.0), b1 = i == 0 ? wb : (i <= k ? wb * yv : 0.0);
        const double a2 = i == 0 ? 1.0 : (i <= k ? ylv : 0.0), b2 = i == 0 ? wl_ : (i <= k ? wl_ * ylv : 0.0);
        const double df = i < k ? (double)y1[ti + fr] - (double)y0[ti + fr] : 0.0;
        d1 = __builtin_amdgcn_mfma_f64_16x16x4f64(a1, b1, d1, 0, 0, 0);
        d2 = __builtin_amdgcn_mfma_f64_16x16x4f64(a2, b2, d2, 0, 0, 0);
        d3 = __builtin_amdgcn_mfma_f64_16x16x4f64(df, wb * df, d3, 0, 0, 0);
      }
      const int cj = lane & 15, o = 1 + k + np;
      const int64_t G = units_x;
#pragma unroll
      for (int r = 0; r < 4; ++r) {
        const int ri = (lane >> 4) + 4 * r;
        int t = -1;
        if (ri == 0 && cj <= k) t = cj;
        else if (ri >= 1 && ri <= cj && cj <= k) {
          const int a_ = ri - 1, b_ = cj - 1;
          t = 1 + k + a_ * k - (a_ * (a_ - 1)) / 2 + (b_ - a_);
        }
        if (t >= 0) partial[t * G + unit] = d1[r];
        if (ri == 0 && cj <= k) partial[(o + cj) * G + unit] = d2[r];
        if (ri >= 1 && ri == cj && cj <= k) partial[(o + 1 + k + (cj - 1)) * G + unit] = d2[r];
        if (ri == cj && cj < k) partial[(o + 1 + 2 * k + cj) * G + unit] = d3[r];
      }
    }
  }
}
}

int cvf_ef_stats_finish_impl(const cvf_ef_cfg* cfg, int n_rows, int stat_major, const double* partial, double* stats,
                             double* loss_vec, double* coef, hipStream_t s);
int cvf_ef_stats_finish_ll(const cvf_ef_cfg* cfg, int n_rows, int stat_major, const double* partial, double* stats,
                           double* loss_vec, double* coef, hipStream_t s, const P2PLL* ll);

static int ef16_units_per_wg(int64_t units, int k, size_t lds_unit_bytes) {
  int cap = 16 / k;
  if (cap > 5) cap = 5;
  while (cap > 1 && (size_t)cap * lds_unit_bytes > 150 * 1024) --cap;
  if (cap < 1) cap = 1;
  int upb = 1;
  (void)units;
  if (const char* e = getenv("CVF_EF16_UPB")) {
    const int v = atoi(e);
    if (v >= 1 && v <= cap) upb = v;
  }
  return upb;
}

template <bool ROWS>
static int ef16_front_go(const char* what, const cvf_mlp_desc* mlp, const float* theta, const float* packed, float* feat_tiled,
                         const cvf_pp_desc* pp, const float* x, int64_t B, const float* a, float* y_tiled, float* saved, float* q_tiled,
                         float* e_tiled, const cvf_ef_cfg* cfg, const float* w, double* scratch, double* stats, double* loss_vec,
                         double* coef, const float* align_rows, void* stream, bool iso = false) {
  CVF_REQUIRE(pp && pp->mode != CVF_PP_FACTORED, "%s: takes coordinates, not CVF_PP_FACTORED records", what);
  CVF_REQUIRE(cvf_ef16_supported(mlp, pp), "%s: shape not covered (cvf_ef16_supported() == 0)", what);
  CVF_REQUIRE(theta && packed && feat_tiled && x && a && y_tiled && saved && q_tiled && e_tiled && cfg && w && scratch && B > 0,
              "%s: bad argument", what);
  CVF_REQUIRE(stats != nullptr || cvf_ef16_rows(B) > 0, "%s: stats == NULL (rows left for cvf_ef16_finish) needs cvf_ef16_rows(B) > 0", what);
  CVF_REQUIRE(cfg->k == mlp->n_nets && cfg->lag_idx == 0, "%s: generator mode only, cfg.k must equal the number of nets", what);
  CVF_REQUIRE(loss_vec == nullptr || coef != nullptr, "%s: loss_vec without coef", what);
  int H, NH;
  ef16_shape(mlp, &H, &NH);
  const int k = mlp->n_nets;
  const int64_t T = cvf_ntiles(B), units = 4 * T;
  const int ns = cvf_ef_nstats(k, 0);
  const bool rows = units <= kMaxRows16;
  const size_t lds1 = (size_t)front16_lds(pp->n_coord, pp->n_align, k).total * sizeof(float);
  const int upb = ef16_units_per_wg(units, k, lds1);
  const size_t lds = lds1 * upb;
  (void)ns;
  ef16_dispatch(H, NH, [&](auto h_, auto nh_) {
    constexpr int kH = decltype(h_)::value, kNH = decltype(nh_)::value;
    auto go = [&](auto kernel) {
      if (lds > 48 * 1024) (void)hipFuncSetAttribute((const void*)kernel, hipFuncAttributeMaxDynamicSharedMemorySize, (int)lds);
      hipLaunchKernelGGL(kernel, dim3((unsigned)((units + upb - 1) / upb)), dim3(64 * k * upb), lds, (hipStream_t)stream, *mlp, theta, packed, *pp,
                         x, B, a, w, feat_tiled, y_tiled, saved, q_tiled, e_tiled, rows ? scratch : nullptr, upb | (iso || cfg->iso_metric != 0 ? 512 : 0), (const float*)nullptr, units,
                         (const float*)nullptr, align_rows);
    };
    const int nit = (pp->n_rec + 3) / 4;
    const bool allal = pp->n_align == pp->n_rec;
#define EF16_GO(NIT_)                                                  \
    case NIT_:                                                          \
      if (allal) go(ef16_front_kernel<kH, kNH, NIT_, true, ROWS>);      \
      else go(ef16_front_kernel<kH, kNH, NIT_, false, ROWS>);           \
      break;
    switch (nit) {
#ifndef CVF_DEV_SHAPES
      EF16_GO(1) EF16_GO(2) EF16_GO(3) EF16_GO(4) EF16_GO(5)
#endif
      default:
        if (allal) go(ef16_front_kernel<kH, kNH, 6, true, ROWS>);
#ifndef CVF_DEV_SHAPES
        else go(ef16_front_kernel<kH, kNH, 6, false, ROWS>);
#endif
    }
#undef EF16_GO
  });
  int rc = cvf_check_launch("ef16_front_kernel");
  if (rc || stats == nullptr) return rc;
  if (rows) return cvf_ef_stats_finish_impl(cfg, (int)units, 1, scratch, stats, loss_vec, coef, (hipStream_t)stream);
  return cvf_ef_stats(cfg, B, w, y_tiled, e_tiled, nullptr, nullptr, scratch, stats, loss_vec, coef, stream);
}
```

Baseline: 353.5 million frames/s.

## Slim front kernel arguments and reorder loads to hide latency

Replaces the large cvf_mlp_desc/cvf_pp_desc kernel arguments with compact Front16Nets/Front16PP structs, so per-layer offsets are computed from compile-time constants instead of loaded from kernel-argument memory. Hoists last-layer weights, hidden fragments and t0 loads to right after layer 0 when the register budget allows, and defers the slow-path x tile load and the y_tiled store so their latency overlaps compute. It also precomputes 3*index addressing and passes a host-computed inv_nal. The cost is higher register pressure in the early-load path, plus a host-side layout check moved into a shared helper.

After: 359.0 million frames/s, median of 6. 1.5% higher.

```diff
diff --git a/colvars-finder_amd/csrc/ef16_back.hip b/colvars-finder_amd/csrc/ef16_back.hip
--- a/colvars-finder_amd/csrc/ef16_back.hip
+++ b/colvars-finder_amd/csrc/ef16_back.hip
@@ -14,10 +14,6 @@
   int n_params;
   int base[CVF_MAX_NETS];
 };
-template <int H, int NH>
-__host__ __device__ constexpr int net_w_off(int l, int hd) { return l == 0 ? 0 : hd + H + (l - 1) * (H * H + H); }
-template <int H, int NH>
-__host__ __device__ constexpr int net_b_off(int l, int hd) { return net_w_off<H, NH>(l, hd) + (l == 0 ? hd : l == NH ? H : H * H); }
 
 template <int H, int NH, bool MULTI, bool GEN>
 __global__ __launch_bounds__(256, 4) void ef16_back_kernel(Back16Args args, Back16Nets nets, const float* __restrict__ theta,
@@ -464,13 +460,7 @@
     covered += span;
   }
   CVF_REQUIRE(covered == mlp->n_params, "cvf_ef16_backward: flat buffer holds parameters outside the nets");
-  for (int n = 0; n < mlp->n_nets; ++n)
-    for (int l = 0; l <= NH; ++l) {
-      CVF_REQUIRE(mlp->b_off[n][l] == mlp->w_off[n][l] + mlp->dims[l] * mlp->dims[l + 1],
-                  "cvf_ef16_backward: net %d, layer %d: the bias does not follow the weight", n, l);
-      CVF_REQUIRE(l == NH || mlp->w_off[n][l + 1] == mlp->b_off[n][l] + mlp->dims[l + 1],
-                  "cvf_ef16_backward: net %d: layer %d does not follow layer %d", n, l + 1, l);
-    }
+  if (ef16_regular_layout("cvf_ef16_backward", mlp, NH)) return -1;
   Back16Nets nets;
   nets.D = mlp->dims[0];
   nets.n_params = mlp->n_params;
diff --git a/colvars-finder_amd/csrc/ef16_common.hpp b/colvars-finder_amd/csrc/ef16_common.hpp
--- a/colvars-finder_amd/csrc/ef16_common.hpp
+++ b/colvars-finder_amd/csrc/ef16_common.hpp
@@ -75,6 +75,32 @@
   return L;
 }
 
+template <int H, int NH>
+__host__ __device__ constexpr int net_w_off(int l, int hd) { return l == 0 ? 0 : hd + H + (l - 1) * (H * H + H); }
+template <int H, int NH>
+__host__ __device__ constexpr int net_b_off(int l, int hd) { return net_w_off<H, NH>(l, hd) + (l == 0 ? hd : l == NH ? H : H * H); }
+
+struct Front16Nets {
+  int D;
+  int k;
+  float inv_nal;
+  int base[CVF_MAX_NETS];
+};
+struct Front16PP {
+  int n_coord, n_align, n_rec;
+  const float* ref_c;
+};
+inline int ef16_regular_layout(const char* what, const cvf_mlp_desc* mlp, int NH) {
+  for (int n = 0; n < mlp->n_nets; ++n)
+    for (int l = 0; l <= NH; ++l) {
+      CVF_REQUIRE(mlp->b_off[n][l] == mlp->w_off[n][l] + mlp->dims[l] * mlp->dims[l + 1],
+                  "%s: net %d, layer %d: the bias does not follow the weight", what, n, l);
+      CVF_REQUIRE(l == NH || mlp->w_off[n][l + 1] == mlp->b_off[n][l] + mlp->dims[l + 1],
+                  "%s: net %d: layer %d does not follow layer %d", what, n, l + 1, l);
+    }
+  return 0;
+}
+
 bool ef16_shape(const cvf_mlp_desc* m, int* H, int* NH) {
   if (m->n_layers < 2 || m->n_layers > 4 || m->dims[m->n_layers] != 1) return false;
   *H = m->dims[1];
diff --git a/colvars-finder_amd/csrc/ef16_front.hip b/colvars-finder_amd/csrc/ef16_front.hip
--- a/colvars-finder_amd/csrc/ef16_front.hip
+++ b/colvars-finder_amd/csrc/ef16_front.hip
@@ -68,6 +68,9 @@
   CVF_REQUIRE(theta && packed && feat_tiled && x && x_lag && y_tiled && saved && B > 0, "%s: bad argument", what);
   int H, NH;
   ef16_shape(mlp, &H, &NH);
+  if (ef16_regular_layout(what, mlp, NH)) return -1;
+  const Front16Nets nets = front16_nets(mlp, pp);
+  const Front16PP ppr = front16_pp(pp);
   const int k = mlp->n_nets;
   const int64_t T = cvf_ntiles(B), units = 4 * T;
   CVF_REQUIRE(2 * units < (int64_t)1 << 31, "%s: batch too large for one launch", what);
@@ -79,8 +82,8 @@
     constexpr int kH = decltype(h_)::value, kNH = decltype(nh_)::value;
     auto kernel = ef16_front_kernel<kH, kNH, 0, true>;
     if (lds > 48 * 1024) (void)hipFuncSetAttribute((const void*)kernel, hipFuncAttributeMaxDynamicSharedMemorySize, (int)lds);
-    hipLaunchKernelGGL(kernel, dim3((unsigned)(paired ? (units + upb - 1) / upb : 2 * units)), dim3(64 * k * upb), lds, (hipStream_t)stream, *mlp,
-                       theta, packed, *pp, x, B, (const float*)nullptr, w, feat_tiled, y_tiled, saved, (float*)nullptr, (float*)nullptr,
+    hipLaunchKernelGGL(kernel, dim3((unsigned)(paired ? (units + upb - 1) / upb : 2 * units)), dim3(front16_block(nets.k, upb)), lds, (hipStream_t)stream, nets,
+                       theta, packed, ppr, x, B, (const float*)nullptr, w, feat_tiled, y_tiled, saved, (float*)nullptr, (float*)nullptr,
                        rows_out, upb | (paired ? 256 : 0), x_lag, units, w_lag, (const float*)nullptr);
   });
   return cvf_check_launch("ef16_front_kernel");
diff --git a/colvars-finder_amd/csrc/ef16_front_kernel.hpp b/colvars-finder_amd/csrc/ef16_front_kernel.hpp
--- a/colvars-finder_amd/csrc/ef16_front_kernel.hpp
+++ b/colvars-finder_amd/csrc/ef16_front_kernel.hpp
@@ -54,8 +54,8 @@
 }
 
 template <int H, int NH, int NIT, bool ALLAL, bool ROWS = false>
-__global__ __launch_bounds__(1024, 4) void ef16_front_kernel(cvf_mlp_desc mlp, const float* __restrict__ theta,
-                                                             const float* __restrict__ packed, cvf_pp_desc pp,
+__global__ __launch_bounds__(1024, 4) void ef16_front_kernel(Front16Nets nets, const float* __restrict__ theta,
+                                                             const float* __restrict__ packed, Front16PP pp,
                                                              const float* __restrict__ x, int64_t B,
                                                              const float* __restrict__ a, const float* __restrict__ w,
                                                              float* __restrict__ feat_tiled, float* __restrict__ y_tiled,
@@ -68,12 +68,12 @@
   constexpr bool kTransfer = NIT == 0;
   extern __shared__ __attribute__((aligned(16))) float lds_all[];
   const int upb = launch & 0xff;
-  const int k = mlp.n_nets, D = mlp.dims[0];
+  const int k = nets.k, D = nets.D;
   const int wave_b = __builtin_amdgcn_readfirstlane((int)threadIdx.x >> 6);
   const int usub = upb > 1 ? wave_b / k : 0;
   const int wave = wave_b - usub * k;
   const int tid = (int)threadIdx.x - usub * (64 * k), lane_in = tid & 63;
-  const int nthreads = upb > 1 ? 64 * k : (int)blockDim.x, nw = nthreads >> 6;
+  const int nthreads = 64 * k, nw = k;
   const int net = wave;
   const int64_t ublock = (int64_t)blockIdx.x * upb + usub;
   const bool paired = kTransfer && x_lag != nullptr && ((launch >> 8) & 1) != 0;
@@ -102,7 +102,9 @@
       for (int rt = 0; rt < RT; ++rt) a0[s][rt] = pk.ld(L.f0() + (se * RT + rt) * 64);
     }
   };
-  auto request_bias0 = [&]() { load_hid_const_u<H>(urows(theta + mlp.b_off[net][0], H, q_), bias[0]); };
+  const float* const th_net = theta + nets.base[net];
+  const int HD = H * D;
+  auto request_bias0 = [&]() { load_hid_const_u<H>(urows(th_net + net_b_off<H, NH>(0, HD), H, q_), bias[0]); };
   auto request_layer0 = [&]() {
     request_a0();
     request_bias0();
@@ -128,6 +130,8 @@
 
   CVF_STAMP(20);
   float bf0[SMAX];
+  constexpr bool kColdLate = RT > 1;
+  bool rows_plain = true;
   if constexpr (ROWS) {
     constexpr int n4r = kRowsUnit / 4;
     const float4* rsrc = reinterpret_cast<const float4*>(rows + unit * (int64_t)kRowsUnit);
@@ -135,6 +139,7 @@
     const float4 row_b = rsrc[tid + nthreads < n4r ? tid + nthreads : n4r - 1];
     const float rs_in = rows[units_x * (int64_t)kRowsUnit + (tid < 3 ? tid : 2)];
     const bool plain = stride == nc && (unit + 1) * kU <= B && (reinterpret_cast<uintptr_t>(x) & 15) == 0;
+    rows_plain = plain;
     const int n4 = (kU * nc) >> 2;
     const float4* xsrc = reinterpret_cast<const float4*>(x + unit * (int64_t)(kU * nc));
     const float4* xs = plain ? xsrc : rsrc;
@@ -170,7 +175,7 @@
       if (tid < n4) dst[tid] = cx0;
       if (tid + nthreads < n4) dst[tid + nthreads] = cx1;
       for (int v = tid + 2 * nthreads; v < n4; v += nthreads) dst[v] = xsrc[v];
-    } else {
+    } else if (!kColdLate) {
       load_x_tile<6>(x, B, nc, unit, xt, tid, nthreads, kU);
     }
     if (tid < nt) refL[tid] = tv;
@@ -229,6 +234,28 @@
   CVF_STAMP(23);
 
   Vec<H, 1> h[NH];
+  constexpr int kFrag = (NH - 1) * NG * RT;
+  constexpr bool kEarly = NG <= 6 && NH * RT * 4 + kFrag + (RT * 4 + kFrag + CTMAX * NG) <= 100;
+  float wl[RT][4];
+  float bL;
+  HFrag<H> tf[NH > 1 ? NH - 1 : 1];
+  float t0[kTransfer ? 1 : CTMAX][NG];
+  auto request_rest = [&]() {
+    load_hid_const_u<H>(urows(th_net + net_w_off<H, NH>(NH, HD), H, q), wl);
+    bL = th_net[net_b_off<H, NH>(NH, HD)];
+    if constexpr (!kTransfer) {
+#pragma unroll
+      for (int l = 1; l < NH; ++l) load_hfrag_u<H>(tf[l - 1], pk, L.th(l));
+#pragma unroll
+      for (int rt = 0; rt < CTMAX; ++rt)
+#pragma unroll
+        for (int s = 0; s < NG; ++s) t0[rt][s] = pk.ld(L.t0() + ((rt < CT ? rt : CT - 1) * NG + s) * 64);
+    }
+    if constexpr (kEarly) {
+      __builtin_amdgcn_sched_barrier(0);
+      asm volatile("" ::: "memory");
+    }
+  };
   auto set_bias = [&](Vec<H, 1>& X, const float (&b)[RT][4]) {
 #pragma unroll
     for (int rt = 0; rt < RT; ++rt)
@@ -253,15 +280,17 @@
       if constexpr (ROWS) bf[s] = bf0[s];
       else bf[s] = fr[kf < D ? kf : D - 1];
     }
+    int S0 = S;
+    asm volatile("" : "+s"(S0));
     HFrag<H> hf[NH > 1 ? NH - 1 : 1];
 #pragma unroll
     for (int l = 1; l < NH; ++l) {
       load_hfrag_u<H>(hf[l - 1], pk, L.fh(l));
-      load_hid_const_u<H>(urows(theta + mlp.b_off[net][l], H, q), bias[l]);
+      load_hid_const_u<H>(urows(th_net + net_b_off<H, NH>(l, HD), H, q), bias[l]);
     }
 #pragma unroll
     for (int s = 0; s < SMAX; ++s) {
-      if (s < S) {
+      if (s == 0 || s < S0) {
 #pragma unroll
         for (int rt = 0; rt < RT; ++rt) h[0].v[rt][0] = mfma4(a0[s][rt], bf[s], h[0].v[rt][0]);
         if constexpr (ROWS) {
@@ -269,6 +298,10 @@
         }
       }
     }
+    if constexpr (ROWS && kColdLate) {
+      if (!iso && !rows_plain) load_x_tile<6>(x, B, nc, unit, xt, tid, nthreads, kU);
+    }
+    if constexpr (kEarly) request_rest();
     CVF_STAMP(24);
     tanh_inplace<H, 1>(h[0]);
 #pragma unroll
@@ -278,30 +311,26 @@
       tanh_inplace<H, 1>(h[l]);
     }
   }
-  float wl[RT][4];
-  load_hid_const_u<H>(urows(theta + mlp.w_off[net][NH], H, q), wl);
-  const float bL = theta[mlp.b_off[net][NH]];
-  HFrag<H> tf[NH > 1 ? NH - 1 : 1];
-#pragma unroll
-  for (int l = 1; l < NH; ++l) load_hfrag_u<H>(tf[l - 1], pk, L.th(l));
-
   const URows sv = urows(saved + (tile * k + net) * (int64_t)(kHand<NH>() * NG * 256) + sub * 64, kHand<NH>() * NG * 256 - sub * 64, lane);
+  if constexpr (!kEarly) request_rest();
+  float yv;
   {
     float part = 0.0f;
 #pragma unroll
     for (int rt = 0; rt < RT; ++rt)
 #pragma unroll
       for (int r = 0; r < 4; ++r) part = fmaf(wl[rt][r], h[NH - 1].v[rt][0][r], part);
-    const float yv = sum_over_q(part) + bL;
+    yv = sum_over_q(part) + bL;
     yL[net * kU + col] = yv;
-    y_tiled[(tile * k + net) * CVF_TILE + kU * sub + col] = yv;
-  }
+  }
+  float* const y_out = y_tiled + (tile * k + net) * CVF_TILE + kU * sub + col;
   CVF_STAMP(25);
   if constexpr (kTransfer) {
 #pragma unroll
     for (int l = 0; l < NH; ++l)
 #pragma unroll
       for (int g = 0; g < NG; ++g) sv.st((l * NG + g) * 256, h[l].v[g >> 2][0][g & 3]);
+    *y_out = yv;
     float* ft = feat_tiled + tile * (int64_t)D * CVF_TILE + kU * sub + f;
     const float* fi = featI + f * kImgP;
 #pragma unroll 1
@@ -310,11 +339,6 @@
   } else {
 
   {
-    float t0[CTMAX][NG];
-#pragma unroll
-    for (int rt = 0; rt < CTMAX; ++rt)
-#pragma unroll
-      for (int s = 0; s < NG; ++s) t0[rt][s] = pk.ld(L.t0() + ((rt < CT ? rt : CT - 1) * NG + s) * 64);
     Vec<H, 1> d;
 #pragma unroll
     for (int rt = 0; rt < RT; ++rt)
@@ -332,7 +356,7 @@
     }
 #pragma unroll
     for (int rt = 0; rt < CTMAX; ++rt) {
-      if (rt < CT) {
+      if ((kEarly && rt == 0) || rt < CT) {
         f32x4 acc = {0.0f, 0.0f, 0.0f, 0.0f};
 #pragma unroll
         for (int s = 0; s < NG; ++s) acc = mfma4(t0[rt][s], d.v[s >> 2][0][s & 3], acc);
@@ -357,18 +381,34 @@
     const float* ar = auxL + f * kAuxP;
     float* Ul = gI + f * kImgP;
     V3 gv[NIT];
+    const int p3 = 3 * p, N3 = 3 * N, nal3 = 3 * nal;
+    auto centred3 = [](const float* my_, int i3, const Centre& c_) {
+      return V3{(my_[i3] - c_.hi[0]) - c_.lo[0], (my_[i3 + 1] - c_.hi[1]) - c_.lo[1], (my_[i3 + 2] - c_.hi[2]) - c_.lo[2]};
+    };
+    auto request_f0b = [&]() {
+      asm volatile("" ::: "memory");
+      int S2 = S;
+      asm volatile("" : "+s"(S2));
+#pragma unroll
+      for (int s_ = 0; s_ < SMAX; ++s_) {
+        const int se = s_ < S2 ? s_ : S2 - 1;
+#pragma unroll
+        for (int rt = 0; rt < RT; ++rt) f0b[s_][rt] = pk.ld(L.f0() + (se * RT + rt) * 64);
+      }
+      __builtin_amdgcn_sched_barrier(0);
+    };
     if (iso) {
     const float* Fl = featI + f * kImgP;
     V3 gsum = v3(0.0f, 0.0f, 0.0f), tau = v3(0.0f, 0.0f, 0.0f);
 #pragma unroll
     for (int it = 0; it < NIT; ++it) {
-      int at = p + 4 * it;
-      asm volatile("" : "+v"(at));
+      int a3 = p3 + 12 * it;
+      asm volatile("" : "+v"(a3));
       const bool last = it == NIT - 1;
-      const int ac = (last && at >= N) ? N - 1 : at;
-      const float lv = (last && at >= N) ? 0.0f : 1.0f;
-      gv[it] = v3(Ul[3 * ac], Ul[3 * ac + 1], Ul[3 * ac + 2]);
-      const V3 fb = v3(Fl[3 * ac], Fl[3 * ac + 1], Fl[3 * ac + 2]);
+      const int c3 = (last && a3 >= N3) ? N3 - 3 : a3;
+      const float lv = (last && a3 >= N3) ? 0.0f : 1.0f;
+      gv[it] = v3(Ul[c3], Ul[c3 + 1], Ul[c3 + 2]);
+      const V3 fb = v3(Fl[c3], Fl[c3 + 1], Fl[c3 + 2]);
       const V3 gm = last ? lv * gv[it] : gv[it];
       gsum = gsum + gm;
       tau.x = fmaf(gm.y, fb.z, fmaf(-gm.z, fb.y, tau.x));
@@ -382,27 +422,27 @@
 #pragma unroll
     for (int i = 0; i < 6; ++i) Kinv[i] = ar[12 + i];
     const V3 s = sym_times(Kinv, tau);
-    const float inv_nal = 1.0f / (float)nal;
+    const float inv_nal = nets.inv_nal;
     const V3 gbar = inv_nal * gsum;
     float E = 0.0f;
     V3 usum = v3(0.0f, 0.0f, 0.0f), tau2 = v3(0.0f, 0.0f, 0.0f);
 #pragma unroll
     for (int it = 0; it < NIT; ++it) {
-      int at = p + 4 * it;
-      asm volatile("" : "+v"(at));
+      int a3 = p3 + 12 * it;
+      asm volatile("" : "+v"(a3));
       const bool last = it == NIT - 1;
-      const int ac = (last && at >= N) ? N - 1 : at;
-      const float lv = (last && at >= N) ? 0.0f : 1.0f;
-      const float ma = ALLAL ? 1.0f : (ac < nal ? 1.0f : 0.0f);
-      const int ar_ = ALLAL ? ac : (ac < nal ? ac : 0);
-      V3 rf = v3(refL[3 * ar_], refL[3 * ar_ + 1], refL[3 * ar_ + 2]);
+      const int c3 = (last && a3 >= N3) ? N3 - 3 : a3;
+      const float lv = (last && a3 >= N3) ? 0.0f : 1.0f;
+      const float ma = ALLAL ? 1.0f : (c3 < nal3 ? 1.0f : 0.0f);
+      const int r3 = ALLAL ? c3 : (c3 < nal3 ? c3 : 0);
+      V3 rf = v3(refL[r3], refL[r3 + 1], refL[r3 + 2]);
       if (!ALLAL) rf = ma * rf;
       const V3 sh = ALLAL ? gbar : ma * gbar;
       V3 G;
       G.x = fmaf(s.y, rf.z, fmaf(-s.z, rf.y, gv[it].x - sh.x));
       G.y = fmaf(s.z, rf.x, fmaf(-s.x, rf.z, gv[it].y - sh.y));
       G.z = fmaf(s.x, rf.y, fmaf(-s.y, rf.x, gv[it].z - sh.z));
-      const V3 u = aL[3 * ac] * G;
+      const V3 u = aL[c3] * G;
       gv[it] = u;
       const bool masked = last || !ALLAL;
       const V3 ue = last ? lv * u : u;
@@ -428,18 +468,18 @@
     CVF_STAMP(31);
 #pragma unroll
     for (int it = 0; it < NIT; ++it) {
-      int at = p + 4 * it;
-      asm volatile("" : "+v"(at));
-      const int ac = (it == NIT - 1 && at >= N) ? N - 1 : at;
-      const V3 fb = v3(Fl[3 * ac], Fl[3 * ac + 1], Fl[3 * ac + 2]);
+      int a3 = p3 + 12 * it;
+      asm volatile("" : "+v"(a3));
+      const int c3 = (it == NIT - 1 && a3 >= N3) ? N3 - 3 : a3;
+      const V3 fb = v3(Fl[c3], Fl[c3 + 1], Fl[c3 + 2]);
       V3 qv;
       qv.x = fmaf(fb.y, om.z, fmaf(-fb.z, om.y, gv[it].x - ubar.x));
       qv.y = fmaf(fb.z, om.x, fmaf(-fb.x, om.z, gv[it].y - ubar.y));
       qv.z = fmaf(fb.x, om.y, fmaf(-fb.y, om.x, gv[it].z - ubar.z));
       gv[it] = qv;
-      Ul[3 * ac] = qv.x;
-      Ul[3 * ac + 1] = qv.y;
-      Ul[3 * ac + 2] = qv.z;
+      Ul[c3] = qv.x;
+      Ul[c3 + 1] = qv.y;
+      Ul[c3 + 2] = qv.z;
     }
     } else {
     float R[9];
@@ -450,15 +490,15 @@
     Outer3 Mo = {{{0.0f, 0.0f}, {0.0f, 0.0f}, {0.0f, 0.0f}}, {0.0f, 0.0f, 0.0f}};
 #pragma unroll
     for (int it = 0; it < NIT; ++it) {
-      int at = p + 4 * it;
-      asm volatile("" : "+v"(at));
+      int a3 = p3 + 12 * it;
+      asm volatile("" : "+v"(a3));
       const bool last = it == NIT - 1;
-      const int ac = (last && at >= N) ? N - 1 : at;
-      const float lv = (last && at >= N) ? 0.0f : 1.0f;
-      gv[it] = v3(Ul[3 * ac], Ul[3 * ac + 1], Ul[3 * ac + 2]);
+      const int c3 = (last && a3 >= N3) ? N3 - 3 : a3;
+      const float lv = (last && a3 >= N3) ? 0.0f : 1.0f;
+      gv[it] = v3(Ul[c3], Ul[c3 + 1], Ul[c3 + 2]);
       const V3 gm = last ? lv * gv[it] : gv[it];
       gsum = gsum + gm;
-      outer_acc(Mo, centred(my, ac, c), gm);
+      outer_acc(Mo, centred3(my, c3, c), gm);
     }
     CVF_STAMP(27);
     gsum = v3(quad_sumf16(gsum.x), quad_sumf16(gsum.y), quad_sumf16(gsum.z));
@@ -482,7 +522,7 @@
       Z[3 * i + 1] = -R[3 * i + 0] * s.z + R[3 * i + 2] * s.x;
       Z[3 * i + 2] = R[3 * i + 0] * s.y - R[3 * i + 1] * s.x;
     }
-    const float inv_nal = 1.0f / (float)nal;
+    const float inv_nal = nets.inv_nal;
     const V3 shift = inv_nal * sump;
     const MatCols Rc = mat_cols(R), Zc = mat_cols(Z);
     f2 E2 = {0.0f, 0.0f};
@@ -492,21 +532,21 @@
     Outer3 dHo = {{{0.0f, 0.0f}, {0.0f, 0.0f}, {0.0f, 0.0f}}, {0.0f, 0.0f, 0.0f}};
 #pragma unroll
     for (int it = 0; it < NIT; ++it) {
-      int at = p + 4 * it;
-      asm volatile("" : "+v"(at));
+      int a3 = p3 + 12 * it;
+      asm volatile("" : "+v"(a3));
       const bool last = it == NIT - 1;
-      const int ac = (last && at >= N) ? N - 1 : at;
-      const float lv = (last && at >= N) ? 0.0f : 1.0f;
-      const float ma = ALLAL ? 1.0f : (ac < nal ? 1.0f : 0.0f);
-      const int ar_ = ALLAL ? ac : (ac < nal ? ac : 0);
-      V3 rf = v3(refL[3 * ar_], refL[3 * ar_ + 1], refL[3 * ar_ + 2]);
+      const int c3 = (last && a3 >= N3) ? N3 - 3 : a3;
+      const float lv = (last && a3 >= N3) ? 0.0f : 1.0f;
+      const float ma = ALLAL ? 1.0f : (c3 < nal3 ? 1.0f : 0.0f);
+      const int r3 = ALLAL ? c3 : (c3 < nal3 ? c3 : 0);
+      V3 rf = v3(refL[r3], refL[r3 + 1], refL[r3 + 2]);
       if (!ALLAL) rf = ma * rf;
       f2 Gxy = ALLAL ? f2{-shift.x, -shift.y} : f2{-ma * shift.x, -ma * shift.y};
       float Gz = ALLAL ? -shift.z : -ma * shift.z;
       mat_times_acc(Rc, gv[it], Gxy, Gz);
       mat_times_acc(Zc, rf, Gxy, Gz);
-      const f2 uxy = f2{aL[3 * ac], aL[3 * ac + 1]} * Gxy;
-      const float uz = aL[3 * ac + 2] * Gz;
+      const f2 uxy = f2{aL[c3], aL[c3 + 1]} * Gxy;
+      const float uz = aL[c3 + 2] * Gz;
       gv[it] = v3(uxy.x, uxy.y, uz);
       const bool masked = last || !ALLAL;
       const float m = ma * lv;
@@ -550,35 +590,36 @@
     const MatRows Rr = mat_rows(R), dRr = mat_rows(dR);
 #pragma unroll
     for (int it = 0; it < NIT; ++it) {
-      int at = p + 4 * it;
-      asm volatile("" : "+v"(at));
-      const int ac = (it == NIT - 1 && at >= N) ? N - 1 : at;
+      int a3 = p3 + 12 * it;
+      asm volatile("" : "+v"(a3));
+      const int c3 = (it == NIT - 1 && a3 >= N3) ? N3 - 3 : a3;
       f2 qxy = {0.0f, 0.0f};
       float qz = 0.0f;
       row_times_acc(Rr, gv[it] - ubar, qxy, qz);
-      row_times_acc(dRr, centred(my, ac, c), qxy, qz);
+      row_times_acc(dRr, centred3(my, c3, c), qxy, qz);
       gv[it] = v3(qxy.x, qxy.y, qz);
-      Ul[3 * ac] = qxy.x;
-      Ul[3 * ac + 1] = qxy.y;
-      Ul[3 * ac + 2] = qz;
+      Ul[c3] = qxy.x;
+      Ul[c3 + 1] = qxy.y;
+      Ul[c3 + 2] = qz;
     }
     }
     CVF_STAMP(32);
-    asm volatile("" ::: "memory");
-#pragma unroll
-    for (int s_ = 0; s_ < SMAX; ++s_) {
-      const int se = s_ < S ? s_ : S - 1;
-#pragma unroll
-      for (int rt = 0; rt < RT; ++rt) f0b[s_][rt] = pk.ld(L.f0() + (se * RT + rt) * 64);
+    request_f0b();
+    {
+      int cy = lane;
+      asm volatile("" : "+v"(cy));
+      if ((cy >> 4) == 0) y_tiled[(tile * k + net) * CVF_TILE + kU * sub + (cy & 15)] = yL[net * kU + (cy & 15)];
     }
     {
       asm volatile("s_waitcnt lgkmcnt(0)" ::: "memory");
       Vec<H, 1> sv0;
       init_bias<H, 1>(sv0, nullptr, q);
       const float* qr = gI + col * kImgP;
+      int S1 = S;
+      asm volatile("" : "+s"(S1));
 #pragma unroll
       for (int s = 0; s < SMAX; ++s) {
-        if (s < S) {
+        if (s == 0 || s < S1) {
           const int kf = 4 * s + q;
           const float b = qr[kf < D ? kf : D - 1];
 #pragma unroll
@@ -592,12 +633,12 @@
     float* qt = q_tiled + (tile * k + net) * (int64_t)D * CVF_TILE + kU * sub + f;
 #pragma unroll
     for (int it = 0; it < NIT; ++it) {
-      int at = p + 4 * it;
-      asm volatile("" : "+v"(at));
-      const int ac = (it == NIT - 1 && at >= N) ? N - 1 : at;
-      qt[(3 * ac) * CVF_TILE] = gv[it].x;
-      qt[(3 * ac + 1) * CVF_TILE] = gv[it].y;
-      qt[(3 * ac + 2) * CVF_TILE] = gv[it].z;
+      int a3 = p3 + 12 * it;
+      asm volatile("" : "+v"(a3));
+      const int c3 = (it == NIT - 1 && a3 >= N3) ? N3 - 3 : a3;
+      qt[c3 * CVF_TILE] = gv[it].x;
+      qt[(c3 + 1) * CVF_TILE] = gv[it].y;
+      qt[(c3 + 2) * CVF_TILE] = gv[it].z;
     }
   }
   CVF_STAMP(34);
@@ -717,6 +758,17 @@
   return upb;
 }
 
+static Front16Nets front16_nets(const cvf_mlp_desc* mlp, const cvf_pp_desc* pp) {
+  Front16Nets n;
+  n.D = mlp->dims[0];
+  n.k = mlp->n_nets;
+  n.inv_nal = 1.0f / (float)pp->n_align;
+  for (int i = 0; i < CVF_MAX_NETS; ++i) n.base[i] = i < mlp->n_nets ? mlp->w_off[i][0] : 0;
+  return n;
+}
+static unsigned front16_block(int k, int upb) { return 64u * (unsigned)k * (unsigned)upb; }
+static Front16PP front16_pp(const cvf_pp_desc* pp) { return Front16PP{pp->n_coord, pp->n_align, pp->n_rec, pp->ref_c}; }
+
 template <bool ROWS>
 static int ef16_front_go(const char* what, const cvf_mlp_desc* mlp, const float* theta, const float* packed, float* feat_tiled,
                          const cvf_pp_desc* pp, const float* x, int64_t B, const float* a, float* y_tiled, float* saved, float* q_tiled,
@@ -731,6 +783,9 @@
   CVF_REQUIRE(loss_vec == nullptr || coef != nullptr, "%s: loss_vec without coef", what);
   int H, NH;
   ef16_shape(mlp, &H, &NH);
+  if (ef16_regular_layout(what, mlp, NH)) return -1;
+  const Front16Nets nets = front16_nets(mlp, pp);
+  const Front16PP ppr = front16_pp(pp);
   const int k = mlp->n_nets;
   const int64_t T = cvf_ntiles(B), units = 4 * T;
   const int ns = cvf_ef_nstats(k, 0);
@@ -743,7 +798,7 @@
     constexpr int kH = decltype(h_)::value, kNH = decltype(nh_)::value;
     auto go = [&](auto kernel) {
       if (lds > 48 * 1024) (void)hipFuncSetAttribute((const void*)kernel, hipFuncAttributeMaxDynamicSharedMemorySize, (int)lds);
-      hipLaunchKernelGGL(kernel, dim3((unsigned)((units + upb - 1) / upb)), dim3(64 * k * upb), lds, (hipStream_t)stream, *mlp, theta, packed, *pp,
+      hipLaunchKernelGGL(kernel, dim3((unsigned)((units + upb - 1) / upb)), dim3(front16_block(nets.k, upb)), lds, (hipStream_t)stream, nets, theta, packed, ppr,
                          x, B, a, w, feat_tiled, y_tiled, saved, q_tiled, e_tiled, rows ? scratch : nullptr, upb | (iso || cfg->iso_metric != 0 ? 512 : 0), (const float*)nullptr, units,
                          (const float*)nullptr, align_rows);
     };
```
